# MasterVVK/qwen3-tts-axera-russian

Measured on AMD Instinct MI355X. Metric: 12Hz codec-tokens/s (codec frames/s, 16 codes each) + RTF, Qwen3-TTS-0.6B, higher is better.
Workload: dtype f16 weights/KV, f32 accumulate (talker+CP); vocoder exact fp32 (f32 MFMA); 1 GPU; configs[2]/[3]: batch=32 mixed ru/en prompts per GPU, 64 frames/utterance/step (prefill + hipGraph decode loop), utterance-sharded DP over 1 GPU(s); batch_per_gpu=32

## Files before the change

include/qwen3tts_engine.h:

```cpp
#ifndef QWEN3TTS_ENGINE_H
#define QWEN3TTS_ENGINE_H

#include <stdint.h>

#ifdef __cplusplus
extern "C" {
#endif

int q3_device_count(void);
int q3_device_compute_units(void);
int q3_set_device(int device);

void* q3e_create(const char* weights, int max_batch, int n_ctx, int max_frames);
void q3e_free(void* e);

int q3e_set_sampling(void* e, float talker_temperature, int talker_top_k, float talker_top_p,
                     float cp_temperature, int cp_top_k, uint64_t seed);

int q3e_set_forced_codes(void* e, const int32_t* forced, int n_frames);

int q3e_set_chains(void* e, int n);

int q3e_set_pad_embed(void* e, const float* pad_embed );

int q3e_start(void* e, int B, const float* prefix, const int32_t* n_rows, const int32_t* n_text,
              int ignore_eos, int max_frames);

int q3e_run(void* e, int n_frames);

float q3e_last_run_ms(void* e);
float q3e_last_prefill_ms(void* e);

int q3e_get_codes(void* e, int32_t* out, int max_out_frames, int32_t* n_frames_per_utt);

int q3e_get_done(void* e, int32_t* done , int32_t* frames );
int q3e_refill(void* e, int n, const int32_t* slots, const float* prefix, const int32_t* n_rows, const int32_t* n_text);

typedef struct q3e_slot_params {
    int32_t max_frames;
    float temperature;
    int32_t top_k;
    float top_p;
    float cp_temperature;
    int32_t cp_top_k;
    uint64_t seed;
    int32_t utt;
    int32_t reserved;
} q3e_slot_params;

int q3e_open(void* e, int B, int ignore_eos);
int q3e_admit(void* e, int n, const int32_t* slots, const float* prefix, const int32_t* n_rows, const int32_t* n_text,
              const q3e_slot_params* params);
int q3e_release(void* e, int n, const int32_t* slots);

int q3e_get_hidden(void* e, float* out);

double q3e_step_weight_bytes(void* e);

#ifdef __cplusplus
}
#endif
#endif
```

qwen3_tts_axera_russian_amd/build.py:

```python
from __future__ import annotations

import os
import shutil
import subprocess
import sys

HERE = os.path.dirname(os.path.abspath(__file__))
CSRC = os.path.join(HERE, "csrc")
LIB = os.path.join(HERE, "lib")
SOURCES = ["q3_common.cpp", "q3_formats.cpp", "q3_kernels.hip", "q3_model.hip", "q3_talker_api.hip", "q3_cp_api.hip",
           "q3_engine.hip", "q3_voc_kernels.hip", "q3_voc.hip", "q3_voc_stream.hip", "q3_enc.hip", "q3_enc_stream.hip",
           "q3_text_api.hip"]
TEST_SOURCES = ["q3_test_api.hip"]
ARCH = os.environ.get("Q3_OFFLOAD_ARCH", "gfx950")
EXTRA = os.environ.get("Q3_EXTRA_HIPCC_FLAGS", "-mllvm -amdgpu-kernarg-preload-count=16").split()


def _newer(dst: str, srcs) -> bool:
    if not os.path.exists(dst):
        return False
    t = os.path.getmtime(dst)
    return all(os.path.getmtime(s) <= t for s in srcs)


NO_SPILL = ("resunit_kernel", "linear_kernelILi1ELi1E", "linear_kernelILi1ELi2E", "linear_kernelILi2ELi1E",
            "linear_kernelILi2ELi2E", "attn_kernel", "attn_short_kernel", "cp_argmax_kernel", "talker_sample_kernel",
            "voc_attn_incr_kernel", "voc_incr_prepend_kernel", "voc_incr_emit_kernel", "voc_incr_prepend_split_kernel",
            "enc_stream_conv_in_kernel", "enc_stream_unfold_kernel", "enc_stream_emit_kernel")


def kernel_resources(lib_path: str):
    import re
    import struct
    import tempfile
    readelf = "/opt/rocm/lib/llvm/bin/llvm-readelf"
    d = open(lib_path, "rb").read()
    res = {}
    i = d.find(b"__CLANG_OFFLOAD_BUNDLE__")
    while i >= 0:
        n = struct.unpack_from("<Q", d, i + 24)[0]
        off = i + 32
        for _ in range(n):
            o, sz, ts = struct.unpack_from("<QQQ", d, off)
            off += 24
            triple = d[off:off + ts].decode()
            off += ts
            if ARCH in triple and sz:
                with tempfile.NamedTemporaryFile(suffix=".elf") as f:
                    f.write(d[i + o:i + o + sz])
                    f.flush()
                    notes = subprocess.run([readelf, "--notes", f.name], capture_output=True, text=True).stdout
                for blk in re.split(r"\n\s+- \.agpr_count:", notes)[1:]:
                    def g(key, blk=blk):
                        m = re.search(r"\." + key + r":\s+(\S+)", blk)
                        return m.group(1) if m else "0"
                    res[g("name")] = (int(g("vgpr_count")), int(blk.split()[0]), int(g("vgpr_spill_count")),
                                      int(g("private_segment_fixed_size")))
        i = d.find(b"__CLANG_OFFLOAD_BUNDLE__", i + 1)
    return res


def check_spills(lib_path: str, verbose: bool = False) -> None:
    if not os.path.exists("/opt/rocm/lib/llvm/bin/llvm-readelf"):
        return
    bad, others = [], []
    for name, (v, a, spill, scratch) in sorted(kernel_resources(lib_path).items()):
        if spill:
            (bad if any(k in name for k in NO_SPILL) else others).append(f"{name}: {spill} spilled VGPRs ({scratch} B scratch)")
    if verbose and others:
        print("kernels with spilled registers (not on the no-spill list):\n  " + "\n  ".join(others), flush=True)
    if bad:
        raise RuntimeError("register spills in kernels that must not spill:\n  " + "\n  ".join(bad))


def build(force: bool = False, verbose: bool = False, timeline: bool = False, refresh_timeline: bool = True) -> str:
    os.makedirs(LIB, exist_ok=True)
    hipcc = shutil.which("hipcc") or "/opt/rocm/bin/hipcc"
    srcs = [os.path.join(CSRC, s) for s in SOURCES if os.path.exists(os.path.join(CSRC, s))]
    hdrs = [os.path.join(CSRC, f) for f in os.listdir(CSRC) if f.endswith(".h")]
    hdrs += [os.path.join(HERE, "..", "include", f) for f in os.listdir(os.path.join(HERE, "..", "include"))]
    tag = "_tl" if timeline else ""
    out = os.path.join(LIB, f"libqwen3tts{tag}.so")
    objs, jobs = [], []
    for s in srcs:
        o = os.path.join(LIB, os.path.basename(s) + tag + ".o")
        objs.append(o)
        if not force and _newer(o, [s] + hdrs):
            continue
        jobs.append([hipcc, f"--offload-arch={ARCH}", "-O3", "-std=c++17", "-fPIC", "-x", "hip", "-c", s, "-o", o,
                     "-Wno-unused-result", "-Wno-unused-value", "-Wno-pass-failed"] + (["-DQ3_TIMELINE"] if timeline else []) + EXTRA)

    def run(cmd):
        if verbose:
            print(" ".join(cmd), flush=True)
        subprocess.check_call(cmd)

    if jobs:
        from concurrent.futures import ThreadPoolExecutor
        with ThreadPoolExecutor(max_workers=min(4, len(jobs))) as pool:
            list(pool.map(run, jobs))
    if force or not _newer(out, objs):
        cmd = [hipcc, f"--offload-arch={ARCH}", "-shared", "-fPIC", "-o", out] + objs + ["-lz"]
        if verbose:
            print(" ".join(cmd), flush=True)
        subprocess.check_call(cmd)
    tout = os.path.join(LIB, f"libqwen3tts_test{tag}.so")
    tsrcs = [os.path.join(CSRC, s) for s in TEST_SOURCES]
    if force or not _newer(tout, tsrcs + hdrs + [out]):
        cmd = [hipcc, f"--offload-arch={ARCH}", "-O3", "-std=c++17", "-fPIC", "-shared", "-x", "hip"] + tsrcs + \
# ... 26 lines not shown
```

qwen3_tts_axera_russian_amd/csrc/q3_cp.h:

```cpp
#pragma once
#include "q3_model.h"

namespace q3 {

struct CpFrameIO {
    int* codes = nullptr;
    const int* n_frames = nullptr;
    int frame_cap = 1;
    float* fb_h = nullptr;
    float* fb_ssq = nullptr;
    half_t* fb_xh = nullptr;
    const float* fb_gamma = nullptr;
    const float* pad_embed = nullptr;
    float temperature = 0.f;
    int top_k = 50;
    unsigned long long seed = 0;
    const unsigned long long* seed_ptr = nullptr;
    const int* forced = nullptr;
    const SlotParams* slots = nullptr;
};

int cp_seed_row0(const Work& w, int R, int row0 = 0, int R_total = 0);
int cp_frame(hipStream_t s, const Model& m, Work& w, KVCache& kv, int R, const CpFrameIO& io, int row0 = 0,
             int R_total = 0);

}
```

qwen3_tts_axera_russian_amd/csrc/q3_cp_api.hip:

```cpp
#include "../../include/qwen3tts_cp.h"
#include "q3_cp.h"

namespace q3 {

static bool two_row_enabled() {
    static const bool on = !(getenv("Q3_CP_TWO_ROW") && atoi(getenv("Q3_CP_TWO_ROW")) == 0);
    return on;
}

int cp_seed_row0(const Work& w, int R, int row0, int R_total) {
    (void)R;
    (void)row0;
    if (R_total <= 0) R_total = R;
    const int B16 = (R_total + 15) / 16 * 16;
    const bool two = two_row_enabled() && 2 * B16 <= w.max_rows;
    return two ? B16 : 0;
}

int cp_frame(hipStream_t s, const Model& m, Work& w, KVCache& kv, int R, const CpFrameIO& io, int row0, int R_total) {
    const ModelCfg& c = m.cfg;
    if (R_total <= 0) R_total = R;
    const int H = c.hidden, G = c.cp_groups;
    const int seed0 = cp_seed_row0(w, R, row0, R_total);
    RowMap rm;
    rm.slot_base = 0;
    rm.slot_stride = 1;
    rm.pos_stride = 0;
    if (seed0 > 0 && (row0 != 0 || R_total != R)) {
        RowMap r0;
        r0.slot_base = -seed0;
        r0.slot_stride = 1;
        r0.pos_base = 0;
        r0.pos_stride = 0;
        r0.same_slot_rows = true;
        if (run_stack(s, m, m.cp, w, kv, R, r0, 256, seed0 + row0)) return -1;
        if (launch_gather_embed(s, m.talker_emb, c.talker_vocab, H, io.codes, 0, io.n_frames, io.frame_cap, 0, w.h, w.ssq, R,
                                row0, R_total, io.forced, w.xh, m.cp.L[0].in_ln))
            return -1;
        RowMap r1 = rm;
        r1.pos_base = 1;
        r1.same_slot_rows = true;
        if (run_stack(s, m, m.cp, w, kv, R, r1, 256, row0)) return -1;
    } else if (seed0 > 0) {
        const int R16 = seed0;
        if (w.map_R16 != R16) {
            std::vector<int> slot(2 * R16), pos(2 * R16);
            for (int i = 0; i < 2 * R16; i++) {
                slot[i] = i % R16;
                pos[i] = i < R16 ? 1 : 0;
            }
            Q3_HIP(hipMemcpyAsync(w.map_slot, slot.data(), sizeof(int) * 2 * R16, hipMemcpyHostToDevice, s), -1);
            Q3_HIP(hipMemcpyAsync(w.map_pos, pos.data(), sizeof(int) * 2 * R16, hipMemcpyHostToDevice, s), -1);
            Q3_HIP(hipStreamSynchronize(s), -1);
            w.map_R16 = R16;
        }
        if (launch_gather_embed(s, m.talker_emb, c.talker_vocab, H, io.codes, 0, io.n_frames, io.frame_cap, 0, w.h, w.ssq, R,
                                row0, R_total, io.forced, w.xh, m.cp.L[0].in_ln))
            return -1;
        RowMap r2;
        r2.slot = w.map_slot;
        r2.pos = w.map_pos;
        r2.same_slot_rows = true;
        r2.valid_mod = R16;
        r2.valid_n = R;
        if (run_stack(s, m, m.cp, w, kv, R16 + R, r2, 256, 0)) return -1;
    } else {
        rm.pos_base = 0;
        if (run_stack(s, m, m.cp, w, kv, R, rm, 256, row0)) return -1;
        if (launch_gather_embed(s, m.talker_emb, c.talker_vocab, H, io.codes, 0, io.n_frames, io.frame_cap, 0, w.h, w.ssq, R,
                                row0, R_total, io.forced, w.xh, m.cp.L[0].in_ln))
            return -1;
        rm.pos_base = 1;
        if (run_stack(s, m, m.cp, w, kv, R, rm, 256, row0)) return -1;
    }
    const bool qkv_tab = m.cp_qkv_serves(R);
    for (int g = 0; g < G; g++) {
        if (g > 0) {
            rm.pos_base = g + 1;
            rm.skip_qkv0 = qkv_tab;
            if (run_stack(s, m, m.cp, w, kv, R, rm, 256, row0)) return -1;
        }
        LinArgs a;
        a.wp = m.cp_head[g].wp;
        a.N = c.cp_vocab;
        a.K = H;
        a.M = row0 + R;
        a.m_begin = row0;
        a.nt = 0;
        a.x16 = w.xh;
        a.ssq = w.ssq;
        a.ssq_parts = H / 16;
        a.eps = c.eps;
        a.y = w.logits;
        a.ldy = c.cp_vocab;
        if (launch_linear(s, a, PRO_NORM, EPI_STORE)) return -1;
        CpArgmaxArgs x;
        x.logits = w.logits;
        x.V = c.cp_vocab;
        x.R = R;
        x.row0 = row0;
        x.R_total = R_total;
        x.H = H;
        x.group = g;
        x.codes = io.codes;
        x.n_frames = io.n_frames;
        x.frame_cap = io.frame_cap;
        x.temperature = io.temperature;
        x.top_k = io.top_k;
        x.seed = io.seed;
        x.seed_ptr = io.seed_ptr;
        x.forced = io.forced;
        x.slots = io.slots;
        if (g + 1 < G) {
            x.next_table = m.cp_emb[g];
            x.h_out = w.h;
            x.ssq_out = w.ssq;
            x.xh_out = w.xh;
            x.gamma_next = m.cp.L[0].in_ln;
            if (qkv_tab) {
                x.next_qkv = m.cp_qkv_rows(g);
                x.qkv_out = w.qkv;
                x.qkv_ld = (c.n_heads + 2 * c.n_kv) * c.head_dim;
            }
        } else if (io.fb_h) {
            x.talker_emb = m.talker_emb;
            x.talker_vocab = c.talker_vocab;
            x.cp_tables = m.d_cp_emb_ptrs;
            x.pad_embed = io.pad_embed;
            x.n_groups = G;
            x.h_out = io.fb_h;
            x.ssq_out = io.fb_ssq;
            x.xh_out = io.fb_xh;
            x.gamma_next = io.fb_gamma;
        }
        if (launch_cp_argmax(s, x)) return -1;
    }
    return 0;
}

}

using namespace q3;

namespace {

struct CpHandle {
    Model* m = nullptr;
    int max_batch = 1;
    KVCache kv;
    Work w;
    hipStream_t s = nullptr;
    int *d_codes = nullptr, *d_nframes = nullptr;
    std::vector<int> h_codes;
    GraphExec graph;
    int graph_rows = 0;
    int step_next_pos = 0;
};

}

extern "C" {

void* cp_load(const char* weights, const char* embeddings_dir, int max_batch) {
    if (!weights) return nullptr;
    if (max_batch <= 0) max_batch = 1;
    hipStream_t s = nullptr;
    if (hipStreamCreate(&s) != hipSuccess) return nullptr;
    Model* m = model_load(weights, false, true, embeddings_dir, s);
    if (!m) {
        hipStreamDestroy(s);
        return nullptr;
    }
    CpHandle* h = new CpHandle();
    h->m = m;
    h->s = s;
    h->max_batch = max_batch;
    const ModelCfg& c = m->cfg;
    bool ok = kv_alloc(h->kv, c.cp_layers, max_batch, c.n_kv, c.cp_groups + 1, h->s) == 0;
// ... 143 lines not shown
```

qwen3_tts_axera_russian_amd/csrc/q3_engine.hip:

```cpp
#include "../../include/qwen3tts_engine.h"
#include "q3_cp.h"

#include <algorithm>
#include <chrono>
#include <cmath>

using namespace q3;

namespace {

struct Engine {
    Model* m = nullptr;
    int max_batch = 0, n_ctx = 0, max_frames = 0;
    hipStream_t s = nullptr;
    KVCache kv_t, kv_c;
    Work wt, wc;
    int prefill_rows = 0;
    int *d_slot = nullptr, *d_pos = nullptr;
    int* d_tiles = nullptr;
    int *d_iota = nullptr;
    int *d_past = nullptr, *d_npast = nullptr, *d_ntext = nullptr, *d_done = nullptr, *d_nframes = nullptr;
    int *d_pos0 = nullptr, *d_posdec = nullptr, *d_lastrow = nullptr;
    int* d_codes = nullptr;
    int* d_forced = nullptr;
// ... 28 lines not shown
    unsigned long long z = seed + golden * k;
    z = (z ^ (z >> 30)) * 0xBF58476D1CE4E5B9ull;
    z = (z ^ (z >> 27)) * 0x94D049BB133111EBull;
    return z ^ (z >> 31);
}

int talker_tail(Engine* e, hipStream_t st, int row0, int R) {
    const Model& m = *e->m;
    const int H = m.cfg.hidden;
    FinalNormArgs f;
    f.h = e->wt.h;
    f.ssq = e->wt.ssq;
    f.ssq_parts = H / 16;
    f.gamma = m.talker.final_norm;
    f.eps = m.cfg.eps;
    f.R = R;
    f.row0 = row0;
    f.H = H;
    f.out_f32 = e->wt.hidden_f32;
    f.out_f16 = e->wt.hidden_f16;
    f.out_copy = e->wc.h;
    f.out_copy_ssq = e->wc.ssq;
    f.out_copy_xh = e->wc.xh;
    f.out_copy_gamma = m.cp.L[0].in_ln;
    f.out_copy_row_off = cp_seed_row0(e->wc, R, row0, e->B);
    if (launch_final_norm(st, f)) return -1;
    LinArgs a;
    a.wp = m.talker_head.wp;
    a.N = m.cfg.talker_vocab;
    a.K = H;
    a.M = row0 + R;
    a.m_begin = row0;
    a.nt = 1;
    a.x16 = e->wt.hidden_f16;
    a.y = e->wt.logits;
    a.ldy = m.cfg.talker_vocab;
    return launch_linear(st, a, PRO_F16, EPI_STORE);
}

int frame_chain(Engine* e, hipStream_t st, int row0, int R) {
    const Model& m = *e->m;
    TalkerSampleArgs sa;
    sa.logits = e->wt.logits;
    sa.V = m.cfg.talker_vocab;
    sa.R = R;
    sa.row0 = row0;
    sa.R_total = e->B;
    sa.audio_vocab = m.cfg.cp_vocab;
    sa.eos = m.cfg.codec_eos;
    sa.past = e->d_past;
    sa.n_past = e->d_npast;
    sa.n_text = e->d_ntext;
    sa.done = e->d_done;
    sa.codes = e->d_codes;
    sa.n_frames = e->d_nframes;
    sa.frame_cap = e->max_frames;
    sa.pos0 = e->d_pos0;
    sa.pos = e->d_posdec;
    sa.ignore_eos = e->ignore_eos;
    sa.max_frames = e->cap_frames;
    sa.temperature = e->t_temp;
    sa.top_k = e->t_top_k;
    sa.top_p = e->t_top_p;
    sa.seed = e->seed;
    sa.seed_ptr = e->d_seed;
    sa.forced = e->forced_on ? e->d_forced : nullptr;
    sa.slots = e->slot_mode ? e->d_slots : nullptr;
    if (launch_talker_sample(st, sa)) return -1;
    CpFrameIO io;
    io.codes = e->d_codes;
    io.n_frames = e->d_nframes;
    io.frame_cap = e->max_frames;
    io.fb_h = e->wt.h;
    io.fb_ssq = e->wt.ssq;
    io.fb_xh = e->wt.xh;
    io.fb_gamma = m.talker.L[0].in_ln;
    io.pad_embed = e->d_pad;
    io.temperature = e->c_temp;
    io.top_k = e->c_top_k;
    io.seed = e->seed ^ 0x5851F42D4C957F2Dull;
    io.seed_ptr = e->d_seed;
    io.forced = e->forced_on ? e->d_forced : nullptr;
    io.slots = e->slot_mode ? e->d_slots : nullptr;
    if (cp_frame(st, m, e->wc, e->kv_c, R, io, row0, e->B)) return -1;
    RowMap rm;
    rm.slot_base = 0;
    rm.slot_stride = 1;
    rm.pos = e->d_posdec;
    rm.rows_total = e->B;
    if (run_stack(st, m, m.talker, e->wt, e->kv_t, R, rm, 1024, row0)) return -1;
    return talker_tail(e, st, row0, R);
}

int n_chains_eff(const Engine* e) {
    const int nc = e->n_chains < 1 ? 1 : e->n_chains;
    return (nc > 1 && e->B % (16 * nc) == 0) ? nc : 1;
}

void chain_rows(const Engine* e, int c, int& row0, int& R) {
    const int nc = n_chains_eff(e);
    row0 = 0;
    for (int i = 0; i < c; i++) row0 += e->B / nc + (i < e->B % nc ? 1 : 0);
    R = e->B / nc + (c < e->B % nc ? 1 : 0);
}

bool make_stream(const Engine* e, hipStream_t* st) {
    return (e->use_prio ? hipStreamCreateWithPriority(st, hipStreamNonBlocking, e->prio_hi)
                        : hipStreamCreateWithFlags(st, hipStreamNonBlocking)) == hipSuccess;
}

int ensure_chains(Engine* e, int n) {
    if (n < 2) return 0;
    if (!e->ev_fork) Q3_HIP(hipEventCreateWithFlags(&e->ev_fork, hipEventDisableTiming), -1);
    for (int c = 0; c < n; c++) {
        if (!e->cs[c] && !make_stream(e, &e->cs[c])) return -1;
        if (!e->ev_join[c]) Q3_HIP(hipEventCreateWithFlags(&e->ev_join[c], hipEventDisableTiming), -1);
    }
    return 0;
}

hipStream_t chain_stream(const Engine* e, int c) { return n_chains_eff(e) == 1 ? e->s : e->cs[c]; }

int frame_eager(Engine* e) {
    const int nc = n_chains_eff(e);
    for (int c = 0; c < nc; c++) {
        int row0, R;
        chain_rows(e, c, row0, R);
        if (frame_chain(e, chain_stream(e, c), row0, R)) return -1;
    }
    return 0;
}

int fork_chains(Engine* e) {
    const int nc = n_chains_eff(e);
    if (nc == 1) return 0;
    Q3_HIP(hipEventRecord(e->ev_fork, e->s), -1);
    for (int c = 0; c < nc; c++) Q3_HIP(hipStreamWaitEvent(e->cs[c], e->ev_fork, 0), -1);
    return 0;
}
int join_chains(Engine* e) {
    const int nc = n_chains_eff(e);
    if (nc == 1) return 0;
    for (int c = 0; c < nc; c++) {
        Q3_HIP(hipEventRecord(e->ev_join[c], e->cs[c]), -1);
        Q3_HIP(hipStreamWaitEvent(e->s, e->ev_join[c], 0), -1);
    }
    return 0;
}

}

extern "C" {

void q3e_free(void* ee) {
    Engine* e = (Engine*)ee;
    if (!e) return;
    if (e->s) hipStreamSynchronize(e->s);
    for (auto& g : e->graph) g.reset();
    kv_free(e->kv_t);
    kv_free(e->kv_c);
    work_free(e->wt);
    work_free(e->wc);
    void* ps[] = {e->d_tiles, e->d_slot, e->d_pos,  e->d_iota,   e->d_past,    e->d_npast, e->d_ntext, e->d_done,
                  e->d_nframes, e->d_pos0, e->d_posdec, e->d_lastrow, e->d_codes, e->d_pad, e->d_forced, e->d_seed, e->d_slots};
    for (void* p : ps)
        if (p) hipFree(p);
// ... 287 lines not shown
    Q3_HIP(hipStreamSynchronize(e->s), -1);
    hipEventElapsedTime(&e->last_prefill_ms, e->ev0, e->ev1);
    return 0;
}

int q3e_run(void* ee, int n_frames) {
    Engine* e = (Engine*)ee;
    if (!e || e->B <= 0 || n_frames <= 0) return -1;
    int room = (e->cap_frames < e->max_frames ? e->cap_frames : e->max_frames) - e->frames_run;
    if (e->slot_mode) {
        room = 0;
        for (int b = 0; b < e->B; b++)
            if (e->h_live[b]) room = std::max(room, e->h_budget[b] - e->h_age[b]);
    }
    if (room <= 0) return 0;
    if (n_frames > room) n_frames = room;
    int done_frames = 0;
    const int nc = n_chains_eff(e);
    Q3_HIP(hipEventRecord(e->ev0, e->s), -1);
    if (fork_chains(e)) return -1;
    static const bool no_graph = getenv("Q3_NO_GRAPH") && atoi(getenv("Q3_NO_GRAPH")) != 0;
    const bool need_capture = !e->graph[0].e || e->graph_B != e->B || e->graph_ignore != e->ignore_eos ||
                              e->graph_cap != e->cap_frames || e->graph_chains != nc ||
                              e->graph_slots != (int)e->slot_mode;
    if (no_graph) {
        for (; done_frames < n_frames; done_frames++)
            if (frame_eager(e)) return -1;
    } else if (need_capture) {
        if (frame_eager(e)) return -1;
        done_frames++;
        for (int c = 0; c < nc; c++) Q3_HIP(hipStreamSynchronize(chain_stream(e, c)), -1);
        for (int c = 0; c < nc; c++) {
            int row0, R;
            chain_rows(e, c, row0, R);
            e->graph[c].reset();
            Q3_HIP(hipStreamBeginCapture(chain_stream(e, c), hipStreamCaptureModeRelaxed), -1);
            int rc = frame_chain(e, chain_stream(e, c), row0, R);
            hipError_t er = hipStreamEndCapture(chain_stream(e, c), &e->graph[c].g);
            if (rc || er != hipSuccess) {
                Q3_LOG("q3e_run: graph capture failed");
                return -1;
            }
            Q3_HIP(hipGraphInstantiate(&e->graph[c].e, e->graph[c].g, nullptr, nullptr, 0), -1);
        }
        e->graph_B = e->B;
        e->graph_ignore = e->ignore_eos;
        e->graph_cap = e->cap_frames;
        e->graph_chains = nc;
        e->graph_slots = (int)e->slot_mode;
    }
    const int check_every = 16;
    const auto th0 = std::chrono::steady_clock::now();
    while (!no_graph && done_frames < n_frames) {
        int chunk = n_frames - done_frames;
        if (!e->ignore_eos && chunk > check_every) chunk = check_every;
        for (int i = 0; i < chunk; i++)
            for (int c = 0; c < nc; c++) Q3_HIP(hipGraphLaunch(e->graph[c].e, chain_stream(e, c)), -1);
        done_frames += chunk;
        if (!e->ignore_eos && done_frames < n_frames) {
            if (join_chains(e)) return -1;
            Q3_HIP(hipMemcpyAsync(e->h_done, e->d_done, sizeof(int) * e->B, hipMemcpyDeviceToHost, e->s), -1);
            Q3_HIP(hipStreamSynchronize(e->s), -1);
            bool all = true;
            for (int b = 0; b < e->B; b++) all = all && e->h_done[b];
            if (all) break;
            if (fork_chains(e)) return -1;
        }
    }
    e->last_host_launch_ms = (float)std::chrono::duration<double, std::milli>(std::chrono::steady_clock::now() - th0).count();
    if (join_chains(e)) return -1;
    Q3_HIP(hipEventRecord(e->ev1, e->s), -1);
    Q3_HIP(hipStreamSynchronize(e->s), -1);
    hipEventElapsedTime(&e->last_run_ms, e->ev0, e->ev1);
    if (e->slot_mode) {
        for (int b = 0; b < e->B; b++)
            if (e->h_age[b] >= 0) e->h_age[b] = std::min(e->h_age[b] + done_frames, e->max_frames);
        return done_frames;
    }
    e->frames_run += done_frames;
    e->frames_hi += done_frames;
    return done_frames;
}

float q3e_last_run_ms(void* ee) { return ee ? ((Engine*)ee)->last_run_ms : -1.f; }
float q3e_last_host_launch_ms(void* ee) { return ee ? ((Engine*)ee)->last_host_launch_ms : -1.f; }
float q3e_last_prefill_ms(void* ee) { return ee ? ((Engine*)ee)->last_prefill_ms : -1.f; }

int q3e_get_codes(void* ee, int32_t* out, int max_out_frames, int32_t* n_frames_per_utt) {
    Engine* e = (Engine*)ee;
    if (!e || !out || e->B <= 0) return -1;
    int nf = e->frames_hi < e->max_frames ? e->frames_hi : e->max_frames;
    if (e->slot_mode) {
        int hi = 0;
        for (int b = 0; b < e->B; b++)
            hi = std::max(hi, e->h_age[b]);
        nf = std::min(hi, e->max_frames);
    }
    if (nf > max_out_frames) nf = max_out_frames;
    int* h_np = e->h_read;
    int* h_codes = e->h_read + e->max_batch;
    const size_t n_codes = 16 * (size_t)e->B * (nf > 0 ? nf : 0);
    if (n_codes) Q3_HIP(hipMemcpyAsync(h_codes, e->d_codes, sizeof(int) * n_codes, hipMemcpyDeviceToHost, e->s), -1);
    if (n_frames_per_utt) Q3_HIP(hipMemcpyAsync(h_np, e->d_npast, sizeof(int) * e->B, hipMemcpyDeviceToHost, e->s), -1);
    Q3_HIP(hipStreamSynchronize(e->s), -1);
    if (n_codes) memcpy(out, h_codes, sizeof(int) * n_codes);
    if (n_frames_per_utt) memcpy(n_frames_per_utt, h_np, sizeof(int) * e->B);
    return nf;
}

int q3e_get_done(void* ee, int32_t* done, int32_t* frames) {
    Engine* e = (Engine*)ee;
    if (!e || !done || e->B <= 0) return -1;
    Q3_HIP(hipMemcpyAsync(e->h_done, e->d_done, sizeof(int) * e->B, hipMemcpyDeviceToHost, e->s), -1);
    Q3_HIP(hipMemcpyAsync(e->h_read, e->d_npast, sizeof(int) * e->B, hipMemcpyDeviceToHost, e->s), -1);
    Q3_HIP(hipStreamSynchronize(e->s), -1);
    memcpy(done, e->h_done, sizeof(int) * e->B);
    std::vector<int> np(e->h_read, e->h_read + e->B);
    for (int b = 0; b < e->B; b++)
        if (np[b] >= (e->slot_mode ? e->h_budget[b] : e->cap_frames)) done[b] = 1;
    if (e->slot_mode)
        for (int b = 0; b < e->B; b++)
            if (done[b]) e->h_live[b] = 0;
    if (frames) memcpy(frames, np.data(), sizeof(int) * e->B);
    return 0;
}

int q3e_refill(void* ee, int n, const int32_t* slots, const float* prefix, const int32_t* n_rows, const int32_t* n_text) {
    Engine* e = (Engine*)ee;
    if (!e || e->B <= 0 || n <= 0 || n > e->B || !slots || !prefix || !n_rows || !n_text) return -1;
    if (e->forced_on) {
        Q3_LOG("q3e_refill: a teacher-forced batch cannot be refilled");
        return -1;
    }
    if (e->slot_mode) {
        Q3_LOG("q3e_refill: a per-slot batch (q3e_open) takes new utterances with q3e_admit");
        return -1;
    }
    std::vector<int> ids(slots, slots + n), seen(e->B, 0);
    for (int u = 0; u < n; u++) {
        const int b = ids[u];
        if (b < 0 || b >= e->B || seen[b]++) {
            Q3_LOG("q3e_refill: slot %d is out of range or listed twice (batch of %d)", b, e->B);
            return -1;
        }
        if (n_rows[u] <= 0 || n_rows[u] > e->prefill_rows || n_rows[u] + e->cap_frames > e->n_ctx) {
            Q3_LOG("q3e_refill: utterance %d: %d prefix rows + %d frames do not fit n_ctx=%d", u, n_rows[u], e->cap_frames, e->n_ctx);
            return -1;
        }
    }
    Q3_HIP(hipStreamSynchronize(e->s), -1);
    Q3_HIP(hipEventRecord(e->ev0, e->s), -1);
    for (int u = 0; u < n; u++) {
        const int b = ids[u];
        if (clear_slot(e, b, n_rows + u, n_text + u)) return -1;
        unsigned long long z = e->req_seed + 0xD1B54A32D192ED03ull * ++e->n_refills;
        z = (z ^ (z >> 30)) * 0xBF58476D1CE4E5B9ull;
        z = (z ^ (z >> 27)) * 0x94D049BB133111EBull;
        z ^= z >> 31;
        Q3_HIP(hipMemcpyAsync(e->d_seed + b, &z, sizeof(z), hipMemcpyHostToDevice, e->s), -1);
        Q3_HIP(hipStreamSynchronize(e->s), -1);
    }
    Q3_HIP(hipStreamSynchronize(e->s), -1);
    if (prefill_ids(e, n, ids.data(), prefix, n_rows, e->B)) return -1;
    if (head_all_rows(e)) return -1;
    Q3_HIP(hipEventRecord(e->ev1, e->s), -1);
    Q3_HIP(hipStreamSynchronize(e->s), -1);
// ... 150 lines not shown
```

qwen3_tts_axera_russian_amd/csrc/q3_kernels.h:

```cpp
#pragma once
#include "q3_common.h"

namespace q3 {

enum { PRO_F16 = 0, PRO_NORM = 1 };
enum { EPI_STORE = 0, EPI_RESID = 1, EPI_SWIGLU = 2 };

struct LinArgs {
    int tl_node = -1;
    const half_t* wp = nullptr;
    int N = 0, K = 0, M = 0;
    int m_begin = 0;
    int swap_grid = 0;
    int nt = 0;
    const half_t* x16 = nullptr;
    const float* ssq = nullptr;
    int ssq_parts = 0;
    float eps = 1e-6f;
    float* y = nullptr;
    int ldy = 0;
    float* h_out = nullptr;
    float* ssq_out = nullptr;
    half_t* xh_out = nullptr;
    const float* gamma = nullptr;
    half_t* act = nullptr;
};
int launch_linear(hipStream_t s, const LinArgs& a, int pro, int epi);
int linear_decode_kbw(int K, int N, int rows);

int launch_pack_linear(hipStream_t s, const half_t* src, int N, int K, half_t* dst, int tile_off,
                       int tile_stride);

enum { ATTN_FUSED = 0, ATTN_PREP = 1, ATTN_ATTEND = 2 };
struct AttnArgs {
    int tl_node = -1;
    float* qkv = nullptr;
    int ld = 0, R = 0, row0 = 0;
    const float* q_norm = nullptr;
    const float* k_norm = nullptr;
    float eps = 1e-6f;
    const float* rope_cos = nullptr;
    const float* rope_sin = nullptr;
    const int* slot = nullptr;
    const int* pos = nullptr;
    int slot_base = 0, slot_stride = 0, pos_base = 0, pos_stride = 0;
    half_t* kc = nullptr;
    half_t* vc = nullptr;
    int n_ctx = 0, n_kv = 0, n_heads = 0;
    half_t* out = nullptr;
    float scale = 0.f;
    int threads = 256;
    int valid_mod = 0, valid_n = 0;
    const int* tiles = nullptr;
    int n_tiles = 0;
};
int launch_attn(hipStream_t s, const AttnArgs& a, int mode);

int launch_ssq_rows(hipStream_t s, const float* rows, float* h, float* ssq, int R, int H, half_t* xh = nullptr,
                    const float* gamma = nullptr, int dst_row0 = 0);

struct FinalNormArgs {
    int tl_node = -1;
    const float* h = nullptr;
    const float* ssq = nullptr;
    int ssq_parts = 0;
    const float* gamma = nullptr;
    float eps = 1e-6f;
    int R = 0, H = 0, row0 = 0;
    const int* row_map = nullptr;
    int src_off = 0;
    float* out_f32 = nullptr;
    half_t* out_f16 = nullptr;
    float* out_copy = nullptr;
    float* out_copy_ssq = nullptr;
    int out_copy_row_off = 0;
    half_t* out_copy_xh = nullptr;
    const float* out_copy_gamma = nullptr;
};
int launch_final_norm(hipStream_t s, const FinalNormArgs& a);

int launch_gather_embed(hipStream_t s, const float* table, int V, int H, const int* tok, int tok_stride,
                        const int* n_frames, int frame_cap, int col, float* h, float* ssq, int R, int row0 = 0,
                        int R_total = 0, const int* forced = nullptr, half_t* xh = nullptr, const float* gamma = nullptr);

struct SlotParams {
    int max_frames = 0;
    float t_temp = 0.f;
    int t_top_k = 0;
    float t_top_p = 1.f;
    float c_temp = 0.f;
    int c_top_k = 0;
    unsigned long long seed = 0;
    int no_row = 1;
    int pad_ = 0;
};

struct TalkerSampleArgs {
    int tl_node = -1;
    const float* logits = nullptr;
    int V = 0, R = 0, row0 = 0, R_total = 0;
    int audio_vocab = 2048, eos = 2150;
    int* past = nullptr;
    int* n_past = nullptr;
    const int* n_text = nullptr;
    int* done = nullptr;
    int* codes = nullptr;
    int* n_frames = nullptr;
    int frame_cap = 0;
    const int* pos0 = nullptr;
    int* pos = nullptr;
    int ignore_eos = 0;
    int max_frames = 0;
    float rep_penalty = 1.2f;
    float temperature = 0.f, top_p = 0.95f;
    int top_k = 50;
    unsigned long long seed = 0;
    const unsigned long long* seed_ptr = nullptr;
    const int* forced = nullptr;
    const SlotParams* slots = nullptr;
};
int launch_talker_sample(hipStream_t s, const TalkerSampleArgs& a);

struct CpArgmaxArgs {
    int tl_node = -1;
    const float* logits = nullptr;
    int V = 0, R = 0, H = 0, row0 = 0, R_total = 0;
    int group = 0;
    int* codes = nullptr;
    const int* n_frames = nullptr;
    int frame_cap = 0;
    const float* next_table = nullptr;
    float* h_out = nullptr;
    float* ssq_out = nullptr;
    half_t* xh_out = nullptr;
    const float* gamma_next = nullptr;
    const float* next_qkv = nullptr;
    float* qkv_out = nullptr;
    int qkv_ld = 0;
// ... 22 lines not shown
```

qwen3_tts_axera_russian_amd/csrc/q3_kernels.hip:

```cpp
#include "q3_kernels.h"

namespace q3 {

typedef _Float16 h8 __attribute__((ext_vector_type(8)));
typedef float f4 __attribute__((ext_vector_type(4)));

#ifdef Q3_TIMELINE
__device__ unsigned long long* g_tl = nullptr;
__device__ unsigned int g_tl_idx = 0;
__device__ unsigned int g_tl_cap = 0;
__device__ int g_skip = 0;
__device__ unsigned long long* g_ph = nullptr;
struct TlScope {
    unsigned int slot = 0xffffffffu;
    int id;
    __device__ __forceinline__ TlScope(int id_) : id(id_) {
        if (blockIdx.x == 0 && blockIdx.y == 0 && threadIdx.x == 0 && g_tl) {
            slot = atomicAdd(&g_tl_idx, 1u);
            if (slot < g_tl_cap) g_tl[2 * slot] = (wall_clock64() << 8) | (unsigned)id;
        }
    }
    __device__ __forceinline__ ~TlScope() {
        if (slot < g_tl_cap) g_tl[2 * slot + 1] = wall_clock64();
    }
};
__device__ unsigned long long* g_tl2 = nullptr;
__device__ int* g_tl2_kind = nullptr;
constexpr int TL2_MAXB = 1024;
struct TlScope2 {
    unsigned long long t0;
    int node, kind;
    __device__ __forceinline__ TlScope2(int n, int k) : node(n), kind(k) { t0 = wall_clock64(); }
    __device__ __forceinline__ ~TlScope2() {
        if (g_tl2 && node >= 0 && threadIdx.x == 0) {
            const unsigned b = blockIdx.x + gridDim.x * blockIdx.y;
            if (b < TL2_MAXB) {
                g_tl2[((size_t)node * TL2_MAXB + b) * 2] = t0;
                g_tl2[((size_t)node * TL2_MAXB + b) * 2 + 1] = wall_clock64();
            }
            if (b == 0 && g_tl2_kind) g_tl2_kind[node] = kind;
        }
    }
};
#define Q3_TL(id)      \
    if (g_skip) return; \
    TlScope2 tl_scope2_(a.tl_node, id); \
    TlScope tl_scope_(id)
#define Q3_PH(n)                                                                                       \
    do {                                                                                               \
        if (tl_scope_.slot < g_tl_cap && g_ph) g_ph[(size_t)tl_scope_.slot * 8 + (n)] = wall_clock64(); \
    } while (0)
#else
#ifndef Q3_WAVE_PRIO
#define Q3_WAVE_PRIO 3
#endif
#if Q3_WAVE_PRIO > 0
#define Q3_TL(id) __builtin_amdgcn_s_setprio(Q3_WAVE_PRIO)
#else
#define Q3_TL(id)
#endif
#define Q3_PH(n)
#endif

#define Q3_FETCH_ARGS(...) asm volatile("" ::__VA_ARGS__)

__device__ __forceinline__ int uniform_load(const int* p) {
    return *(const __attribute__((address_space(4))) int*)p;
}

__device__ __forceinline__ float wave_sum(float v) {
#pragma unroll
    for (int o = 32; o > 0; o >>= 1) v += __shfl_xor(v, o, 64);
    return v;
}
__device__ __forceinline__ float wave_max(float v) {
#pragma unroll
    for (int o = 32; o > 0; o >>= 1) v = fmaxf(v, __shfl_xor(v, o, 64));
    return v;
}
__device__ __forceinline__ half_t sat_half(float x) {
    return (half_t)fminf(fmaxf(x, -65504.f), 65504.f);
}
constexpr float NORM_PRE = 0.0625f, NORM_POST = 16.0f;
#ifdef Q3_NT_OUT
#define Q3_OUT_STORE(v_, p_) __builtin_nontemporal_store((v_), (p_))
#else
#define Q3_OUT_STORE(v_, p_) (*(p_) = (v_))
#endif
__device__ __forceinline__ half_t pre_scaled(float h, float g) { return sat_half((h * g) * NORM_PRE); }

__device__ __forceinline__ size_t frag_idx(int m, int k, int K) {
    return ((((size_t)(m >> 4) * (K >> 5) + (k >> 5)) * 64 + (m & 15) + 16 * ((k >> 3) & 3)) << 3) + (k & 7);
}

__global__ void pack_linear_kernel(const half_t* __restrict__ src, int N, int K, half_t* __restrict__ dst,
                                   int tile_off, int tile_stride) {
    const int KB = K / 32;
    size_t idx = (size_t)blockIdx.x * blockDim.x + threadIdx.x;
    size_t total = (size_t)(N / 16) * KB * 64;
    if (idx >= total) return;
    int lane = (int)(idx & 63);
    size_t blk = idx >> 6;
    int kb = (int)(blk % KB);
    int ts = (int)(blk / KB);
    int n = ts * 16 + (lane & 15);
    int k = kb * 32 + (lane >> 4) * 8;
    h8 v = *(const h8*)(src + (size_t)n * K + k);
    size_t td = (size_t)tile_off + (size_t)ts * tile_stride;
    *(h8*)(dst + ((td * KB + kb) * 64 + lane) * 8) = v;
}

int launch_pack_linear(hipStream_t s, const half_t* src, int N, int K, half_t* dst, int tile_off,
                       int tile_stride) {
    if (N % 16 || K % 32) {
        Q3_LOG("pack_linear: N=%d K=%d not multiples of 16/32", N, K);
        return -1;
    }
    size_t total = (size_t)(N / 16) * (K / 32) * 64;
    int blocks = (int)((total + 255) / 256);
    hipLaunchKernelGGL(pack_linear_kernel, dim3(blocks), dim3(256), 0, s, src, N, K, dst, tile_off, tile_stride);
    Q3_HIP(hipGetLastError(), -1);
    return 0;
}

static const char* g_last_variant = "";
const char* last_linear_variant() { return g_last_variant; }
static const char* pro_name(int pro) { return pro == PRO_NORM ? "NORM" : "F16"; }
static const char* epi_name(int epi) { return epi == EPI_STORE ? "STORE" : epi == EPI_RESID ? "RESID" : "SWIGLU"; }
static int env_int(const char* name, int dflt) { return getenv(name) ? atoi(getenv(name)) : dflt; }

template <int NB16, int MT16, int KBW, int NW, int PRO, int EPI, bool NT>
__global__ void __launch_bounds__(NW * 64)
    linear_kernel(const half_t* __restrict__ p_wp, const void* __restrict__ p_asrc, const float* __restrict__ p_ssq,
                  const float* __restrict__ p_gamma, void* __restrict__ p_out, int p_M, int p_N, int p_m_begin,
                  int p_swap, float p_eps, LinArgs a) {
    a.wp = p_wp;
    a.x16 = (const half_t*)p_asrc;
    a.ssq = p_ssq;
    a.gamma = p_gamma;
    a.y = (float*)p_out;
    a.h_out = (float*)p_out;
    a.act = (half_t*)p_out;
    a.M = p_M;
    a.N = p_N;
    a.m_begin = p_m_begin;
    a.swap_grid = p_swap;
    a.eps = p_eps;
    constexpr int MR = MT16 * 16, NB = NB16 * 16, NBP = NB + 4, KB = NW * KBW, K = KB * 32;
    constexpr int NTH = NW * 64;
    constexpr int NOUT = (EPI == EPI_SWIGLU) ? MR * NB / 2 : MR * NB;
    constexpr int OPT = (NOUT + NTH - 1) / NTH;
    constexpr int SQI = (MR * 16 + NTH - 1) / NTH;
    Q3_TL(10 + PRO * 4 + EPI);
    const int tid = threadIdx.x, lane = tid & 63, w = tid >> 6;
    const int q = lane >> 4, c = lane & 15;
    const int tile0 = (a.swap_grid ? blockIdx.y : blockIdx.x) * NB16;
    const int m0 = a.m_begin + (a.swap_grid ? blockIdx.x : blockIdx.y) * MR;
    extern __shared__ __attribute__((aligned(16))) char smem[];
    float* red = (float*)smem;
    float* inv_s = red + NW * MR * NBP;

    float4 sq[SQI];
    h8 af[MT16][KBW];
    float hold[OPT], gnext[OPT];
    if (PRO == PRO_NORM) {
#pragma unroll
        for (int i = 0; i < SQI; i++) {
            const int g4 = tid + i * NTH, g4c = g4 < MR * 16 ? g4 : 0;
            sq[i] = *(const float4*)(a.ssq + (size_t)(m0 + g4c / 16) * 64 + (g4c & 15) * 4);
        }
    }
    if (EPI == EPI_RESID) {
#pragma unroll
        for (int i = 0; i < OPT; i++) {
            const int o = tid + i * NTH;
            const int m = m0 + o / NB;
            hold[i] = 0.f;
            gnext[i] = 0.f;
            if (o < NOUT && m < a.M) hold[i] = a.h_out[frag_idx(m, tile0 * 16 + (o % NB), a.N)];
            if (o < NOUT && a.gamma) gnext[i] = a.gamma[tile0 * 16 + (o % NB)];
        }
    }
    h8 wf[NB16][KBW];
#pragma unroll
    for (int nb = 0; nb < NB16; nb++)
#pragma unroll
        for (int kbi = 0; kbi < KBW; kbi++) {
            const h8* p = (const h8*)(a.wp + (((size_t)(tile0 + nb) * KB + (size_t)w * KBW + kbi) * 64 + lane) * 8);
            wf[nb][kbi] = NT ? __builtin_nontemporal_load(p) : *p;
        }
#pragma unroll
    for (int kbi = 0; kbi < KBW; kbi++) {
        const int k0 = (w * KBW + kbi) * 32 + q * 8;
#pragma unroll
        for (int mt = 0; mt < MT16; mt++) {
            af[mt][kbi] = *(const h8*)(a.x16 + frag_idx(m0 + mt * 16 + c, k0, K));
        }
    }
    __builtin_amdgcn_sched_barrier(0);
    if (EPI == EPI_RESID) Q3_FETCH_ARGS("s"(a.ssq_out), "s"(a.xh_out));
    if (EPI == EPI_STORE) Q3_FETCH_ARGS("s"(a.ldy));
    if (PRO == PRO_NORM) Q3_FETCH_ARGS("s"(a.eps));
    Q3_PH(0);

    if (PRO == PRO_NORM) {
#pragma unroll
        for (int i = 0; i < SQI; i++) {
            const int g4 = tid + i * NTH;
            float s = (sq[i].x + sq[i].y) + (sq[i].z + sq[i].w);
            s += __shfl_xor(s, 8, 16);
            s += __shfl_xor(s, 4, 16);
            s += __shfl_xor(s, 2, 16);
            s += __shfl_xor(s, 1, 16);
            if (g4 < MR * 16 && (g4 & 15) == 0) inv_s[g4 / 16] = (1.0f / sqrtf(s / (float)K + a.eps)) * NORM_POST;
        }
    }

    Q3_PH(1);
    f4 acc[MT16][NB16];
#pragma unroll
    for (int mt = 0; mt < MT16; mt++)
#pragma unroll
        for (int nb = 0; nb < NB16; nb++) acc[mt][nb] = (f4){0.f, 0.f, 0.f, 0.f};
#pragma unroll
    for (int kbi = 0; kbi < KBW; kbi++)
#pragma unroll
        for (int mt = 0; mt < MT16; mt++)
#pragma unroll
            for (int nb = 0; nb < NB16; nb++)
                acc[mt][nb] = __builtin_amdgcn_mfma_f32_16x16x32_f16(af[mt][kbi], wf[nb][kbi], acc[mt][nb], 0, 0, 0);

    asm volatile("" ::"v"(acc[0][0][0]));
    Q3_PH(2);
#define RED(w_, row_, col_) red[((w_) * MR + (row_)) * NBP + (col_)]
#pragma unroll
    for (int mt = 0; mt < MT16; mt++)
#pragma unroll
        for (int nb = 0; nb < NB16; nb++)
#pragma unroll
            for (int r = 0; r < 4; r++) RED(w, mt * 16 + 4 * q + r, nb * 16 + c) = acc[mt][nb][r];
    __syncthreads();
    Q3_PH(3);

    if (EPI == EPI_STORE || EPI == EPI_RESID) {
#pragma unroll
        for (int i = 0; i < OPT; i++) {
            const int o = tid + i * NTH;
            if (o < NOUT) {
                const int mr = o / NB, n = o % NB;
                float v = 0.f;
#pragma unroll
                for (int ww = 0; ww < NW; ww++) v += RED(ww, mr, n);
                const int m = m0 + mr;
                const int ng = tile0 * 16 + n;
                const bool ok = m < a.M;
                if (PRO == PRO_NORM) v *= inv_s[mr];
                if (EPI == EPI_STORE) {
                    if (ok) Q3_OUT_STORE(v, &a.y[(size_t)m * a.ldy + ng]);
                } else {
                    const float hn = ok ? hold[i] + v : 0.f;
                    if (ok) Q3_OUT_STORE(hn, &a.h_out[frag_idx(m, ng, a.N)]);
                    if (ok && a.xh_out) Q3_OUT_STORE(pre_scaled(hn, gnext[i]), &a.xh_out[frag_idx(m, ng, a.N)]);
                    float s = hn * hn;
                    s += __shfl_xor(s, 8, 16);
                    s += __shfl_xor(s, 4, 16);
                    s += __shfl_xor(s, 2, 16);
                    s += __shfl_xor(s, 1, 16);
                    if (ok && (n & 15) == 0) Q3_OUT_STORE(s, &a.ssq_out[(size_t)m * (a.N / 16) + (ng >> 4)]);
                }
            }
        }
    } else {
        constexpr int NH = NB / 2;
#pragma unroll
        for (int i = 0; i < OPT; i++) {
            const int o = tid + i * NTH;
            if (o < NOUT) {
                const int mr = o / NH, j = o % NH;
                const int ii = j >> 4, cc = j & 15;
                float g = 0.f, u = 0.f;
#pragma unroll
                for (int ww = 0; ww < NW; ww++) {
                    g += RED(ww, mr, (2 * ii) * 16 + cc);
                    u += RED(ww, mr, (2 * ii + 1) * 16 + cc);
                }
                const int m = m0 + mr;
                if (PRO == PRO_NORM) {
                    g *= inv_s[mr];
                    u *= inv_s[mr];
                }
                if (m < a.M) {
                    const float sg = __fdividef(g, 1.0f + __expf(-g));
                    Q3_OUT_STORE(sat_half(sg * u), &a.act[frag_idx(m, (tile0 / NB16) * NH + j, a.N / 2)]);
                }
            }
        }
    }
#undef RED
}

template <int NB16, int MT16, int KBW, int NW, int PRO, int EPI, bool NT>
static int launch_linear_nt(hipStream_t s, const LinArgs& a) {
    constexpr int MR = MT16 * 16, NBP = NB16 * 16 + 4;
    constexpr size_t lds = (size_t)NW * MR * NBP * 4 + MR * 4;
    static bool attr_set = false;
    if (!attr_set) {
        if (lds > 48 * 1024)
            Q3_HIP(hipFuncSetAttribute((const void*)linear_kernel<NB16, MT16, KBW, NW, PRO, EPI, NT>,
                                       hipFuncAttributeMaxDynamicSharedMemorySize, (int)lds), -1);
        attr_set = true;
    }
    static char name[64];
    if (!name[0])
        snprintf(name, sizeof(name), "linear<%d,%d,%d,%d,%s,%s,%s>", NB16, MT16, KBW, NW, pro_name(PRO), epi_name(EPI), NT ? "nt" : "t");
    g_last_variant = name;
    LinArgs b = a;
    b.tl_node = tl_next_node();
    const unsigned nt_ = a.N / (16 * NB16), nr_ = (a.M - a.m_begin + MR - 1) / MR;
    b.swap_grid = nr_ > 2 ? 1 : 0;
    dim3 grid(b.swap_grid ? nr_ : nt_, b.swap_grid ? nt_ : nr_);
    const void* asrc = (const void*)b.x16;
    void* outp = EPI == EPI_STORE ? (void*)b.y : EPI == EPI_RESID ? (void*)b.h_out : (void*)b.act;
    hipLaunchKernelGGL((linear_kernel<NB16, MT16, KBW, NW, PRO, EPI, NT>), grid, dim3(NW * 64), lds, s, b.wp, asrc, b.ssq,
                       b.gamma, outp, b.M, b.N, b.m_begin, b.swap_grid, b.eps, b);
    Q3_HIP(hipGetLastError(), -1);
    return 0;
}

__device__ __forceinline__ void gemm_tile_of_block(int R, int T, int& row_tile, int& col_tile) {
    const int L = blockIdx.x;
    if (T % 8 == 0) {
        const int x = L & 7, j = L >> 3;
        row_tile = j % R;
        col_tile = x + 8 * (j / R);
    } else {
        row_tile = L % R;
        col_tile = L / R;
    }
}

template <int BM, int BN, int PRO, int EPI>
__device__ __forceinline__ void gemm_epilogue(const LinArgs& a, f4 (&acc)[BM / 32][BN / 32], const float* post, int m0,
                                              int tile0, int wm, int wn, int q, int c) {
    constexpr int WM = BM / 32, WN = BN / 32;
#pragma unroll
    for (int i = 0; i < WM; i++) {
#pragma unroll
        for (int r = 0; r < 4; r++) {
            const int mr = (wm * WM + i) * 16 + 4 * q + r;
            const int m = m0 + mr;
            const bool ok = m < a.M;
            const float ps = PRO == PRO_NORM ? post[mr] : 1.0f;
            if (EPI == EPI_SWIGLU) {
#pragma unroll
                for (int j = 0; j < WN; j += 2) {
                    const float g = acc[i][j][r] * ps, u = acc[i][j + 1][r] * ps;
                    const float sg = __fdividef(g, 1.0f + __expf(-g));
                    const int jn = ((tile0 + wn * WN + j) >> 1) * 16 + c;
                    if (ok) a.act[frag_idx(m, jn, a.N / 2)] = sat_half(sg * u);
                }
            } else {
#pragma unroll
                for (int j = 0; j < WN; j++) {
                    const int ng = (tile0 + wn * WN + j) * 16 + c;
                    const float v = acc[i][j][r] * ps;
                    if (EPI == EPI_STORE) {
                        if (ok) a.y[(size_t)m * a.ldy + ng] = v;
                    } else {
                        const size_t hi = frag_idx(m, ng, a.N);
                        const float hn = ok ? a.h_out[hi] + v : 0.f;
                        if (ok) a.h_out[hi] = hn;
                        if (ok && a.xh_out) a.xh_out[hi] = pre_scaled(hn, a.gamma[ng]);
                        float s2 = hn * hn;
                        s2 += __shfl_xor(s2, 8, 16);
                        s2 += __shfl_xor(s2, 4, 16);
                        s2 += __shfl_xor(s2, 2, 16);
                        s2 += __shfl_xor(s2, 1, 16);
                        if (ok && c == 0) a.ssq_out[(size_t)m * (a.N / 16) + (ng >> 4)] = s2;
                    }
                }
            }
        }
    }
}

template <int BM, int BN, int KS, int PRO, int EPI>
__global__ void __launch_bounds__(256) gemm_kernel(LinArgs a) {
    constexpr int RA = BM / 16, RB = BN / 16;
    constexpr int NF = (RA + RB) * KS, FPW = NF / 4;
    constexpr int WM = BM / 32, WN = BN / 32;
    static_assert(NF % 4 == 0 && WN % 2 == 0, "tile shape");
    Q3_TL(20 + PRO * 4 + EPI);
    const int tid = threadIdx.x, lane = tid & 63, w = tid >> 6;
    const int wm = w >> 1, wn = w & 1, q = lane >> 4, c = lane & 15;
    int row_tile, col_tile;
    gemm_tile_of_block((a.M - a.m_begin + BM - 1) / BM, a.N / BN, row_tile, col_tile);
    const int m0 = a.m_begin + row_tile * BM;
    const int tile0 = col_tile * RB;
    const int KB = a.K >> 5, NST = KB / KS;
    extern __shared__ __attribute__((aligned(16))) char smem[];
    h8* lds = (h8*)smem;
    __shared__ float post[BM];
    if (PRO == PRO_NORM) {
        for (int r = tid; r < BM; r += 256) {
            const int m = m0 + r;
// ... 302 lines not shown
        for (int kbi = 0; kbi < KBW; kbi++)
            af[kbi] = *(const h8*)(p_x16 + frag_idx(blk0 + c, (w * KBW + kbi) * 32 + q * 8, K));
    }
    __builtin_amdgcn_sched_barrier(0);
    Q3_PH(0);
    f4 acc = (f4){0.f, 0.f, 0.f, 0.f};
#pragma unroll
    for (int kbi = 0; kbi < KBW; kbi++) acc = __builtin_amdgcn_mfma_f32_16x16x32_f16(af[kbi], wf[kbi], acc, 0, 0, 0);
    Q3_PH(2);
    if ((q >> 1) == half) *(f4*)(red + ((w * 2 + (q & 1)) * 16 + c) * 4) = acc;
    __syncthreads();
    Q3_PH(3);
    if (epi_thread) {
        float v = 0.f;
#pragma unroll
        for (int ww = 0; ww < NW; ww++) v += red[((ww * 2 + (mr >> 2)) * 16 + n) * 4 + (mr & 3)];
        const float hn = ok ? hold + v : 0.f;
        if (ok) Q3_OUT_STORE(hn, &p_h[frag_idx(m, ng, N)]);
        if (ok && p_xh_out) Q3_OUT_STORE(pre_scaled(hn, gnext), &p_xh_out[frag_idx(m, ng, N)]);
        float s = hn * hn;
        s += __shfl_xor(s, 8, 16);
        s += __shfl_xor(s, 4, 16);
        s += __shfl_xor(s, 2, 16);
        s += __shfl_xor(s, 1, 16);
        if (ok && n == 0) Q3_OUT_STORE(s, &p_ssq_out[(size_t)m * (N / 16) + tile0]);
    }
}

static int g_narrow8 = env_int("Q3_LINEAR_NARROW8", 1);
int set_linear_narrow8(int on) { g_narrow8 = on; return 0; }

template <int KBW, int NW>
static int launch_linear_narrow_t(hipStream_t s, const LinArgs& a) {
    const int groups = (a.M - a.m_begin + 7) / 8;
    const int node = tl_next_node();
    static char name[2][32];
    if (!name[0][0]) {
        snprintf(name[0], sizeof(name[0]), "narrow<%d,%d,t>", KBW, NW);
        snprintf(name[1], sizeof(name[1]), "narrow<%d,%d,nt>", KBW, NW);
    }
    g_last_variant = name[a.nt ? 1 : 0];
    if (a.nt)
        hipLaunchKernelGGL((linear_narrow_kernel<KBW, NW, true>), dim3(64, groups), dim3(NW * 64), 0, s, a.wp, a.x16, a.h_out, a.gamma,
                           a.ssq_out, a.xh_out, a.M, a.m_begin, node);
    else
        hipLaunchKernelGGL((linear_narrow_kernel<KBW, NW, false>), dim3(64, groups), dim3(NW * 64), 0, s, a.wp, a.x16, a.h_out, a.gamma,
                           a.ssq_out, a.xh_out, a.M, a.m_begin, node);
    Q3_HIP(hipGetLastError(), -1);
    return 0;
}

#define Q3_LIN_CASE(NB16_, MT16_, KBW_, NW_, PRO_, EPI_)                                   \
    if (nb16 == NB16_ && mt16 == MT16_ && kbw == KBW_ && nw == NW_ && pro == PRO_ && epi == EPI_) \
        return launch_linear_t<NB16_, MT16_, KBW_, NW_, PRO_, EPI_>(s, a);

#define Q3_LIN_MT(NB16_, KBW_, NW_, PRO_, EPI_) \
    Q3_LIN_CASE(NB16_, 1, KBW_, NW_, PRO_, EPI_) \
    Q3_LIN_CASE(NB16_, 2, KBW_, NW_, PRO_, EPI_) \
    Q3_LIN_CASE(NB16_, 4, KBW_, NW_, PRO_, EPI_)

int reset_linear_knobs() {
    memcpy(g_tune_kbw, g_tune_kbw_default, sizeof(g_tune_kbw));
    g_wide_tiles = 0;
    g_split_rows_narrow = 1;
    g_gemm_min_rows = 65;
    g_narrow8 = env_int("Q3_LINEAR_NARROW8", 1);
    g_gemm_glds = env_int("Q3_GEMM_GLDS", 1);
    return 0;
}

static int decode_mt16(int rows, int N) {
    int mt16 = rows <= 16 ? 1 : rows <= 32 ? 2 : 4;
    if (rows > 16 && rows <= 32 && ((g_split_rows_narrow == 1 && N <= 1024) || g_split_rows_narrow == 2)) mt16 = 1;
    return mt16;
}

int linear_decode_kbw(int K, int N, int rows) {
    const int ki = K == 1024 ? 0 : K == 2048 ? 1 : K == 3072 ? 2 : -1;
    if (rows <= 0 || rows >= g_gemm_min_rows || ki < 0 || N % 32) return 0;
    const int mt16 = decode_mt16(rows, N);
    return g_tune_kbw[ki][mt16 == 1 ? 0 : mt16 == 2 ? 1 : 2];
}

int launch_linear(hipStream_t s, const LinArgs& a, int pro, int epi) {
    g_last_variant = "";
    const int rows = a.M - a.m_begin;
    if (rows <= 0) return 0;
    if (rows >= g_gemm_min_rows) return launch_gemm(s, a, pro, epi);
    const int K = a.K;
    int ki = K == 1024 ? 0 : K == 2048 ? 1 : K == 3072 ? 2 : -1;
    if (ki < 0 || a.N % 32) {
        Q3_LOG("launch_linear: unsupported shape N=%d K=%d", a.N, K);
        return -1;
    }
    if (g_narrow8 && pro == PRO_F16 && epi == EPI_RESID && a.N == 1024 && a.m_begin % 16 == 0 && a.ssq_out) {
        if (K == 2048) return launch_linear_narrow_t<16, 4>(s, a);
        if (K == 3072) return launch_linear_narrow_t<12, 8>(s, a);
    }
    const int mt16 = decode_mt16(rows, a.N);
    const int kbw = g_tune_kbw[ki][mt16 == 1 ? 0 : mt16 == 2 ? 1 : 2];
    const int nw = K / 32 / kbw;
    const int nb16 = (epi == EPI_SWIGLU || (g_wide_tiles && rows > 16 && K == 1024 && epi == EPI_STORE)) ? 2 : 1;
    Q3_LIN_MT(1, 8, 4, PRO_NORM, EPI_STORE)
    Q3_LIN_MT(1, 4, 8, PRO_NORM, EPI_STORE)
    Q3_LIN_MT(2, 8, 4, PRO_NORM, EPI_SWIGLU)
    Q3_LIN_MT(2, 4, 8, PRO_NORM, EPI_SWIGLU)
    Q3_LIN_MT(1, 8, 4, PRO_F16, EPI_STORE)
    Q3_LIN_MT(2, 4, 8, PRO_NORM, EPI_STORE)
    Q3_LIN_MT(2, 4, 8, PRO_F16, EPI_STORE)
    Q3_LIN_MT(1, 4, 8, PRO_F16, EPI_STORE)
    Q3_LIN_MT(1, 8, 8, PRO_F16, EPI_RESID)
    Q3_LIN_MT(1, 4, 16, PRO_F16, EPI_RESID)
    Q3_LIN_MT(1, 16, 4, PRO_F16, EPI_RESID)
    Q3_LIN_MT(1, 6, 16, PRO_F16, EPI_RESID)
    Q3_LIN_MT(1, 12, 8, PRO_F16, EPI_RESID)
    Q3_LOG("launch_linear: no instantiation for K=%d kbw=%d nw=%d mt16=%d nb16=%d pro=%d epi=%d", K, kbw, nw,
           mt16, nb16, pro, epi);
    return -1;
}

__device__ __forceinline__ void store_row_ssq(float* h, float* ssq, int r, int H, int k4, float4 v,
                                              half_t* xh = nullptr, const float* gamma = nullptr) {
    *(float4*)(h + frag_idx(r, k4 * 4, H)) = v;
    if (xh) {
        const float4 g = *(const float4*)(gamma + k4 * 4);
        half_t* p = xh + frag_idx(r, k4 * 4, H);
        p[0] = pre_scaled(v.x, g.x);
        p[1] = pre_scaled(v.y, g.y);
        p[2] = pre_scaled(v.z, g.z);
        p[3] = pre_scaled(v.w, g.w);
    }
    float s = v.x * v.x + v.y * v.y + v.z * v.z + v.w * v.w;
    s += __shfl_xor(s, 1, 4);
    s += __shfl_xor(s, 2, 4);
    if ((k4 & 3) == 0) ssq[(size_t)r * (H / 16) + (k4 >> 2)] = s;
}

__global__ void ssq_rows_kernel(const float* __restrict__ rows, float* __restrict__ h, float* __restrict__ ssq, int H,
                                half_t* __restrict__ xh, const float* __restrict__ gamma, int dst_row0) {
    const int r = blockIdx.x;
    for (int k4 = threadIdx.x; k4 < H / 4; k4 += blockDim.x)
        store_row_ssq(h, ssq, dst_row0 + r, H, k4, *(const float4*)(rows + (size_t)r * H + k4 * 4), xh, gamma);
}
int launch_ssq_rows(hipStream_t s, const float* rows, float* h, float* ssq, int R, int H, half_t* xh, const float* gamma,
                    int dst_row0) {
    if (R <= 0) return 0;
    hipLaunchKernelGGL(ssq_rows_kernel, dim3(R), dim3(256), 0, s, rows, h, ssq, H, xh, gamma, dst_row0);
    Q3_HIP(hipGetLastError(), -1);
    return 0;
}

__global__ void final_norm_kernel(FinalNormArgs a) {
    Q3_FETCH_ARGS("s"(a.h), "s"(a.ssq), "s"(a.ssq_parts), "s"(a.gamma), "s"(a.eps), "s"(a.H), "s"(a.row0), "s"(a.row_map), "s"(a.src_off),
                  "s"(a.out_f32), "s"(a.out_f16), "s"(a.out_copy), "s"(a.out_copy_ssq), "s"(a.out_copy_xh), "s"(a.out_copy_gamma),
                  "s"(a.out_copy_row_off));
    Q3_TL(40);
    __shared__ float inv_sh;
    const int r = a.row0 + blockIdx.x;
    const int src = a.row_map ? uniform_load(a.row_map + r) : r + a.src_off;
    if (threadIdx.x < 64) {
        float s = 0.f;
        for (int p = threadIdx.x; p < a.ssq_parts; p += 64) s += a.ssq[(size_t)src * a.ssq_parts + p];
        s = wave_sum(s);
        if (threadIdx.x == 0) inv_sh = 1.0f / sqrtf(s / (float)a.H + a.eps);
    }
    __syncthreads();
    const float iv = inv_sh;
    for (int k4 = threadIdx.x; k4 < a.H / 4; k4 += blockDim.x) {
        const float4 v = *(const float4*)(a.h + frag_idx(src, k4 * 4, a.H));
        const float4 g = *(const float4*)(a.gamma + k4 * 4);
        float4 o;
        o.x = (v.x * iv) * g.x;
        o.y = (v.y * iv) * g.y;
        o.z = (v.z * iv) * g.z;
        o.w = (v.w * iv) * g.w;
        if (a.out_f32) *(float4*)(a.out_f32 + (size_t)r * a.H + k4 * 4) = o;
        if (a.out_f16) {
            half_t* p = a.out_f16 + frag_idx(r, k4 * 4, a.H);
            p[0] = sat_half(o.x);
            p[1] = sat_half(o.y);
            p[2] = sat_half(o.z);
            p[3] = sat_half(o.w);
        }
        if (a.out_copy)
            store_row_ssq(a.out_copy, a.out_copy_ssq, r + a.out_copy_row_off, a.H, k4, o, a.out_copy_xh, a.out_copy_gamma);
    }
}
int launch_final_norm(hipStream_t s, const FinalNormArgs& a) {
    if (a.R <= 0) return 0;
    FinalNormArgs a2 = a;
    a2.tl_node = tl_next_node();
    hipLaunchKernelGGL(final_norm_kernel, dim3(a.R), dim3(256), 0, s, a2);
    Q3_HIP(hipGetLastError(), -1);
    return 0;
}

__global__ void gather_embed_kernel(const float* __restrict__ table, int V, int H, const int* __restrict__ tok,
                                    int tok_stride, const int* __restrict__ n_frames, int frame_cap, int col,
                                    float* __restrict__ h, float* __restrict__ ssq, int row0, int R_total,
                                    const int* __restrict__ forced, half_t* __restrict__ xh,
                                    const float* __restrict__ gamma) {
    const int r = row0 + blockIdx.x;
    int t;
// ... 152 lines not shown
        l1 = l1 * c1 + p1;
#pragma unroll
        for (int j = 0; j < 8; j++) {
            const float vf = (float)vv[j];
            a0[j] = a0[j] * c0 + p0 * vf;
            a1[j] = a1[j] * c1 + p1 * vf;
        }
        m0 = n0;
        m1 = n1;
    };
#pragma unroll
    for (int i = 0; i < APRE; i++) {
        const int t = grp + i * ngrp;
        if (t < T) step(kpre[i], vpre[i]);
    }
#pragma unroll 2
    for (int t = grp + APRE * ngrp; t < T; t += ngrp) {
        const h8 kk = *(const h8*)(kbase + (size_t)t * D + l16 * 8);
        const h8 vv = *(const h8*)(vbase + (size_t)t * D + l16 * 8);
        step(kk, vv);
    }
    if (MODE == ATTN_FUSED && grp == 0) {
        h8 kk, vv;
#pragma unroll
        for (int j = 0; j < 8; j++) {
            kk[j] = (half_t)knew[l16 * 8 + j];
            vv[j] = (half_t)vnew[l16 * 8 + j];
        }
        step(kk, vv);
    }
    asm volatile("" ::"v"(a0[0]), "v"(l0));
    Q3_PH(2);
#pragma unroll
    for (int o = 16; o <= 32; o <<= 1) {
        const float om0 = __shfl_xor(m0, o, 64), om1 = __shfl_xor(m1, o, 64);
        const float ol0 = __shfl_xor(l0, o, 64), ol1 = __shfl_xor(l1, o, 64);
        const float n0 = fmaxf(m0, om0), n1 = fmaxf(m1, om1);
        const float c0 = (m0 == -INFINITY) ? 0.f : __expf(m0 - n0), d0 = (om0 == -INFINITY) ? 0.f : __expf(om0 - n0);
        const float c1 = (m1 == -INFINITY) ? 0.f : __expf(m1 - n1), d1 = (om1 == -INFINITY) ? 0.f : __expf(om1 - n1);
        l0 = l0 * c0 + ol0 * d0;
        l1 = l1 * c1 + ol1 * d1;
#pragma unroll
        for (int j = 0; j < 8; j++) {
            const float oa0 = __shfl_xor(a0[j], o, 64), oa1 = __shfl_xor(a1[j], o, 64);
            a0[j] = a0[j] * c0 + oa0 * d0;
            a1[j] = a1[j] * c1 + oa1 * d1;
        }
        m0 = n0;
        m1 = n1;
    }
    if (lane < 16) {
#pragma unroll
        for (int j = 0; j < 8; j++) {
            pacc[(w * 2 + 0) * D + lane * 8 + j] = a0[j];
            pacc[(w * 2 + 1) * D + lane * 8 + j] = a1[j];
        }
        if (lane == 0) {
            pm[w * 2 + 0] = m0;
            pm[w * 2 + 1] = m1;
            pl[w * 2 + 0] = l0;
            pl[w * 2 + 1] = l1;
        }
    }
    __syncthreads();
    Q3_PH(3);
    if (tid < 2 * D) {
        const int hh = tid / D, d = tid % D;
        float M = -INFINITY;
        for (int i = 0; i < nwv; i++) M = fmaxf(M, pm[i * 2 + hh]);
        float L = 0.f, o = 0.f;
        for (int i = 0; i < nwv; i++) {
            const float mi = pm[i * 2 + hh];
            const float c = (mi == -INFINITY) ? 0.f : __expf(mi - M);
            L += pl[i * 2 + hh] * c;
            o += pacc[(i * 2 + hh) * D + d] * c;
        }
        a.out[frag_idx(r, (2 * g + hh) * D + d, a.n_heads * D)] = sat_half(o / L);
    }
}

constexpr int ATTN_SHORT_MAX_T = 15;
static int g_attn_short = 1;
int set_attn_short(int on) { g_attn_short = on; return 0; }
__global__ void __launch_bounds__(256)
    attn_short_kernel(float* __restrict__ p_qkv, int p_ld, int p_row0, int p_n_heads, int p_n_kv,
                      const float* __restrict__ p_q_norm, const float* __restrict__ p_k_norm,
                      const float* __restrict__ p_rope_cos, const float* __restrict__ p_rope_sin, int p_pos_base,
                      int p_slot_base, AttnArgs a) {
    constexpr int D = 128, NE = ATTN_SHORT_MAX_T + 1;
    a.qkv = p_qkv;
    a.ld = p_ld;
    a.row0 = p_row0;
    a.n_heads = p_n_heads;
    a.n_kv = p_n_kv;
    a.q_norm = p_q_norm;
    a.k_norm = p_k_norm;
    a.rope_cos = p_rope_cos;
    a.rope_sin = p_rope_sin;
    a.pos_base = p_pos_base;
    a.slot_base = p_slot_base;
    Q3_FETCH_ARGS("s"(a.eps), "s"(a.slot), "s"(a.slot_stride), "s"(a.kc), "s"(a.vc), "s"(a.n_ctx), "s"(a.out), "s"(a.scale));
    Q3_TL(33);
    const int r = a.row0 + blockIdx.x, g = blockIdx.y;
    const int tid = threadIdx.x, lane = tid & 63, w = tid >> 6;
    const int slot = a.slot ? uniform_load(a.slot + r) : a.slot_base + r * a.slot_stride;
    const int T = a.pos_base;
    __shared__ float qs[2][D];
    __shared__ float knew[D];
    __shared__ __attribute__((aligned(16))) half_t vs[NE][D];
    __shared__ __attribute__((aligned(16))) float sc[2][NE];
    float* row = a.qkv + (size_t)r * a.ld;
    const size_t cbase = ((size_t)slot * a.n_kv + g) * (size_t)a.n_ctx * D;
    const int l16 = tid & 15, grp = tid >> 4;
    const int hh = tid >> 7, d = tid & 127;
    float x0 = 0.f, x1 = 0.f, gm0 = 1.f, gm1 = 1.f, cs = 1.f, sn = 0.f;
    {
        const float* src = w < 2 ? row + (size_t)(2 * g + w) * D
                         : w == 2 ? row + (size_t)(a.n_heads + g) * D
                                  : row + (size_t)(a.n_heads + a.n_kv + g) * D;
        x0 = src[lane];
        x1 = src[lane + 64];
        if (w < 3) {
            const float* gam = w < 2 ? a.q_norm : a.k_norm;
            gm0 = gam[lane];
            gm1 = gam[lane + 64];
            cs = a.rope_cos[(size_t)T * 64 + lane];
            sn = a.rope_sin[(size_t)T * 64 + lane];
        }
    }
    h8 kpre, vpre;
    if (grp < T) {
        kpre = *(const h8*)(a.kc + cbase + (size_t)grp * D + l16 * 8);
        vpre = *(const h8*)(a.vc + cbase + (size_t)grp * D + l16 * 8);
    }
    __builtin_amdgcn_sched_barrier(0);
    Q3_PH(0);
    if (w < 3) {
        float ss = wave_sum(x0 * x0 + x1 * x1);
        const float iv = 1.0f / sqrtf(ss / (float)D + a.eps);
        x0 = (x0 * iv) * gm0;
        x1 = (x1 * iv) * gm1;
        const float y0 = x0 * cs - x1 * sn;
        const float y1 = x1 * cs + x0 * sn;
        x0 = y0;
        x1 = y1;
    }
    if (w < 2) {
        qs[w][lane] = x0;
        qs[w][lane + 64] = x1;
    } else {
        const half_t h0 = sat_half(x0), h1 = sat_half(x1);
        half_t* cd = (w == 2 ? a.kc : a.vc) + cbase + (size_t)T * D;
        cd[lane] = h0;
        cd[lane + 64] = h1;
        if (w == 2) {
            knew[lane] = (float)h0;
            knew[lane + 64] = (float)h1;
        } else {
            vs[T][lane] = h0;
            vs[T][lane + 64] = h1;
        }
    }
    if (grp < T) *(h8*)(&vs[grp][l16 * 8]) = vpre;
    __syncthreads();
    Q3_PH(1);
    if (grp <= T) {
        float d0 = 0.f, d1 = 0.f;
#pragma unroll
        for (int j = 0; j < 8; j++) {
            const float kf = grp < T ? (float)kpre[j] : knew[l16 * 8 + j];
            d0 += (qs[0][l16 * 8 + j] * a.scale) * kf;
            d1 += (qs[1][l16 * 8 + j] * a.scale) * kf;
        }
#pragma unroll
        for (int o = 8; o > 0; o >>= 1) {
            d0 += __shfl_xor(d0, o, 16);
            d1 += __shfl_xor(d1, o, 16);
        }
        if (l16 == 0) {
            sc[0][grp] = d0;
            sc[1][grp] = d1;
        }
    }
    __syncthreads();
    Q3_PH(2);
    float sv[NE];
#pragma unroll
    for (int e4 = 0; e4 < NE; e4 += 4) {
        const float4 t4 = *(const float4*)(&sc[hh][e4]);
        sv[e4] = t4.x;
        sv[e4 + 1] = t4.y;
        sv[e4 + 2] = t4.z;
        sv[e4 + 3] = t4.w;
    }
    float m = -INFINITY;
#pragma unroll
    for (int e = 0; e < NE; e++) m = fmaxf(m, e <= T ? sv[e] : -INFINITY);
    float L = 0.f, o = 0.f;
#pragma unroll
    for (int e = 0; e < NE; e++) {
        const float p = e <= T ? __expf(sv[e] - m) : 0.f;
        const float vf = e <= T ? (float)vs[e][d] : 0.f;
        L += p;
        o += p * vf;
    }
    Q3_PH(3);
    a.out[frag_idx(r, (2 * g + hh) * D + d, a.n_heads * D)] = sat_half(o / L);
}

__global__ void __launch_bounds__(256) attn_tile_mfma_kernel(AttnArgs a) {
    constexpr int D = 128, QP = 136, VP = 72, CH = 64;
    constexpr float LO = 2048.0f, ILO = 1.0f / 2048.0f;
    Q3_TL(35);
    const int g = blockIdx.y, tid = threadIdx.x, lane = tid & 63, w = tid >> 6;
    const int c = lane & 15, q4 = lane >> 4;
    int row0, nrows, slot, pos0;
    if (a.tiles) {
        const int4 t = *(const int4*)(a.tiles + 4 * blockIdx.x);
        row0 = t.x; nrows = t.y; slot = t.z; pos0 = t.w;
    } else {
        row0 = a.row0 + blockIdx.x * 16;
        nrows = a.R - blockIdx.x * 16 < 16 ? a.R - blockIdx.x * 16 : 16;
        slot = a.slot_base;
        pos0 = a.pos_base + blockIdx.x * 16;
    }
    extern __shared__ __attribute__((aligned(16))) char smem[];
    half_t* qh = (half_t*)smem;
    half_t* ql = qh + 32 * QP;
    half_t* ks = ql + 32 * QP;
    half_t* vs = ks + CH * QP;
    half_t* ph = vs + CH * QP;
    half_t* pl = ph + 32 * VP;
    float* red = (float*)(pl + 32 * VP);
    float* red2 = red + 4 * 32;
    const size_t cbase = ((size_t)slot * a.n_kv + g) * (size_t)a.n_ctx * D;
    const int T = pos0 + nrows;
    h8 kreg[4], vreg[4];
    auto load_chunk = [&](int c0) {
#pragma unroll
        for (int it = 0; it < 4; it++) {
            const int idx = tid + it * 256, kr = idx >> 4, d8 = (idx & 15) * 8;
            kreg[it] = vreg[it] = (h8){0, 0, 0, 0, 0, 0, 0, 0};
            if (c0 + kr < T) {
                kreg[it] = *(const h8*)(a.kc + cbase + (size_t)(c0 + kr) * D + d8);
                vreg[it] = *(const h8*)(a.vc + cbase + (size_t)(c0 + kr) * D + d8);
            }
        }
    };
    auto store_chunk = [&]() {
#pragma unroll
        for (int it = 0; it < 4; it++) {
            const int idx = tid + it * 256, kr = idx >> 4, d8 = (idx & 15) * 8;
            *(h8*)(ks + kr * QP + d8) = kreg[it];
            *(h8*)(vs + kr * QP + d8) = vreg[it];
        }
    };
    load_chunk(0);
    for (int idx = tid; idx < 32 * (D / 8); idx += 256) {
        const int qr = idx / (D / 8), d8 = (idx - qr * (D / 8)) * 8, i = qr & 15, hh = qr >> 4;
        h8 hi = {0, 0, 0, 0, 0, 0, 0, 0}, lo = hi;
        if (i < nrows) {
            const float* src = a.qkv + (size_t)(row0 + i) * a.ld + (size_t)(2 * g + hh) * D + d8;
            const float4 v0 = *(const float4*)src, v1 = *(const float4*)(src + 4);
            const float e[8] = {v0.x, v0.y, v0.z, v0.w, v1.x, v1.y, v1.z, v1.w};
#pragma unroll
            for (int j = 0; j < 8; j++) {
                const float x = e[j] * a.scale;
                hi[j] = sat_half(x);
                lo[j] = (half_t)((x - (float)hi[j]) * LO);
            }
        }
        *(h8*)(qh + qr * QP + d8) = hi;
        *(h8*)(ql + qr * QP + d8) = lo;
    }
    float mrow[2][4], lrow[2][4];
    f4 oh[2][2], ol[2][2];
#pragma unroll
    for (int qb = 0; qb < 2; qb++)
#pragma unroll
        for (int r = 0; r < 4; r++) {
            mrow[qb][r] = -INFINITY;
            lrow[qb][r] = 0.f;
        }
#pragma unroll
    for (int qb = 0; qb < 2; qb++)
#pragma unroll
        for (int j = 0; j < 2; j++) oh[qb][j] = ol[qb][j] = (f4){0.f, 0.f, 0.f, 0.f};
    for (int c0 = 0; c0 < T; c0 += CH) {
        __syncthreads();
        store_chunk();
// ... 31 lines not shown
                if (c == 0) red[w * 32 + 16 * qb + i] = x;
            }
        __syncthreads();
        float corr[2][4];
#pragma unroll
        for (int qb = 0; qb < 2; qb++)
#pragma unroll
            for (int r = 0; r < 4; r++) {
                const int qr = 16 * qb + 4 * q4 + r;
                const float cm = fmaxf(fmaxf(red[qr], red[32 + qr]), fmaxf(red[64 + qr], red[96 + qr]));
                const float mo = mrow[qb][r], mn = fmaxf(mo, cm);
                corr[qb][r] = (mo == -INFINITY) ? 0.f : __expf(mo - mn);
                const float p = (sc[qb][r] == -INFINITY) ? 0.f : __expf(sc[qb][r] - mn);
                const half_t hi = (half_t)p;
                ph[qr * VP + 16 * w + c] = hi;
                pl[qr * VP + 16 * w + c] = (half_t)((p - (float)hi) * LO);
                float ssum = p;
                ssum += __shfl_xor(ssum, 1, 16);
                ssum += __shfl_xor(ssum, 2, 16);
                ssum += __shfl_xor(ssum, 4, 16);
                ssum += __shfl_xor(ssum, 8, 16);
                if (c == 0) red2[w * 32 + qr] = ssum;
                mrow[qb][r] = mn;
            }
        __syncthreads();
#pragma unroll
        for (int qb = 0; qb < 2; qb++)
#pragma unroll
            for (int r = 0; r < 4; r++) {
                const int qr = 16 * qb + 4 * q4 + r;
                lrow[qb][r] = lrow[qb][r] * corr[qb][r] + ((red2[qr] + red2[32 + qr]) + (red2[64 + qr] + red2[96 + qr]));
#pragma unroll
                for (int j = 0; j < 2; j++) {
                    oh[qb][j][r] *= corr[qb][r];
                    ol[qb][j][r] *= corr[qb][r];
                }
            }
#pragma unroll
        for (int kst = 0; kst < 2; kst++) {
#pragma unroll
            for (int j = 0; j < 2; j++) {
                typedef __fp16 hv4 __attribute__((__vector_size__(4 * sizeof(__fp16))));
                const half_t* vb = vs + (kst * 32 + 8 * q4 + (c >> 2)) * QP + 32 * w + 16 * j + 4 * (c & 3);
                const hv4 t0 = __builtin_amdgcn_ds_read_tr16_b64_v4f16((__attribute__((address_space(3))) hv4*)vb);
                const hv4 t1 = __builtin_amdgcn_ds_read_tr16_b64_v4f16((__attribute__((address_space(3))) hv4*)(vb + 4 * QP));
                h8 bv;
#pragma unroll
                for (int e = 0; e < 4; e++) {
                    bv[e] = (half_t)t0[e];
                    bv[4 + e] = (half_t)t1[e];
                }
#pragma unroll
                for (int qb = 0; qb < 2; qb++) {
                    const h8 ahi = *(const h8*)(ph + (16 * qb + c) * VP + kst * 32 + q4 * 8);
                    const h8 alo = *(const h8*)(pl + (16 * qb + c) * VP + kst * 32 + q4 * 8);
                    oh[qb][j] = __builtin_amdgcn_mfma_f32_16x16x32_f16(ahi, bv, oh[qb][j], 0, 0, 0);
                    ol[qb][j] = __builtin_amdgcn_mfma_f32_16x16x32_f16(alo, bv, ol[qb][j], 0, 0, 0);
                }
            }
        }
    }
#pragma unroll
    for (int qb = 0; qb < 2; qb++)
#pragma unroll
        for (int r = 0; r < 4; r++) {
            const int i = 4 * q4 + r;
            if (i < nrows) {
                const float inv = 1.0f / lrow[qb][r];
#pragma unroll
                for (int j = 0; j < 2; j++) {
                    const float o = (oh[qb][j][r] + ol[qb][j][r] * ILO) * inv;
                    a.out[frag_idx(row0 + i, (2 * g + qb) * D + 32 * w + 16 * j + c, a.n_heads * D)] = sat_half(o);
                }
            }
        }
}

int launch_attn(hipStream_t s, const AttnArgs& a, int mode) {
    if (a.R <= 0) return 0;
    if (a.n_heads != 2 * a.n_kv) {
        Q3_LOG("attn: only GQA group 2 (16q/8kv) is built, got %d/%d", a.n_heads, a.n_kv);
        return -1;
    }
    if (g_attn_short && mode == ATTN_FUSED && !a.pos && a.pos_stride == 0 && a.pos_base >= 0 &&
        a.pos_base <= ATTN_SHORT_MAX_T && a.pos_base < a.n_ctx) {
        AttnArgs a3 = a;
        a3.tl_node = tl_next_node();
        hipLaunchKernelGGL(attn_short_kernel, dim3(a.R, a.n_kv), dim3(256), 0, s, a3.qkv, a3.ld, a3.row0, a3.n_heads, a3.n_kv,
                           a3.q_norm, a3.k_norm, a3.rope_cos, a3.rope_sin, a3.pos_base, a3.slot_base, a3);
        Q3_HIP(hipGetLastError(), -1);
        return 0;
    }
    if (mode == ATTN_ATTEND && a.n_tiles > 0) {
        constexpr size_t lds = (size_t)(2 * 32 * 136 + 2 * 64 * 136 + 2 * 32 * 72) * 2 + 8 * 32 * 4;
        static bool attr = false;
        if (!attr) {
            Q3_HIP(hipFuncSetAttribute((const void*)attn_tile_mfma_kernel, hipFuncAttributeMaxDynamicSharedMemorySize, (int)lds), -1);
            attr = true;
        }
        AttnArgs a5 = a;
        a5.tl_node = tl_next_node();
        hipLaunchKernelGGL(attn_tile_mfma_kernel, dim3(a.n_tiles, a.n_kv), dim3(256), lds, s, a5);
        Q3_HIP(hipGetLastError(), -1);
        return 0;
    }
    int threads = a.threads;
    const int fit = 65536 / (a.R * a.n_kv);
    if (threads > fit) threads = fit / 64 * 64;
    if (threads < 256) threads = 256;
    if (threads > 1024) threads = 1024;
    const size_t lds = ((size_t)(threads / 64) * (4 + 2 * 128)) * sizeof(float);
    AttnArgs a2 = a;
    a2.tl_node = tl_next_node();
    dim3 grid(a.R, a.n_kv);
#define Q3_ATTN(MODE_)                                                                                   \
    {                                                                                                    \
        if (threads <= 256)                                                                              \
            hipLaunchKernelGGL((attn_kernel<MODE_, 8>), grid, dim3(256), mode == ATTN_PREP ? 0 : lds, s, a2); \
        else                                                                                             \
            hipLaunchKernelGGL((attn_kernel<MODE_, 4>), grid, dim3(mode == ATTN_PREP ? 256 : threads),   \
                               mode == ATTN_PREP ? 0 : lds, s, a2);                                      \
    }
    if (mode == ATTN_FUSED) Q3_ATTN(ATTN_FUSED)
    else if (mode == ATTN_PREP) Q3_ATTN(ATTN_PREP)
    else Q3_ATTN(ATTN_ATTEND)
#undef Q3_ATTN
    Q3_HIP(hipGetLastError(), -1);
    return 0;
}

__device__ __forceinline__ void block_argmax(float& v, int& idx, float* sv, int* si) {
#pragma unroll
    for (int o = 32; o > 0; o >>= 1) {
        const float ov = __shfl_xor(v, o, 64);
        const int oi = __shfl_xor(idx, o, 64);
        if (ov > v || (ov == v && oi < idx)) {
            v = ov;
            idx = oi;
        }
    }
    const int w = threadIdx.x >> 6, nw = blockDim.x >> 6;
    if ((threadIdx.x & 63) == 0) {
        sv[w] = v;
        si[w] = idx;
    }
    __syncthreads();
    v = sv[0];
    idx = si[0];
    for (int i = 1; i < nw; i++)
        if (sv[i] > v || (sv[i] == v && si[i] < idx)) {
            v = sv[i];
            idx = si[i];
        }
    __syncthreads();
}

__device__ __forceinline__ float uniform01(unsigned long long seed, unsigned row, unsigned frame, unsigned group) {
    unsigned long long z = seed + 0x9E3779B97F4A7C15ull * (1ull + row + ((unsigned long long)frame << 20) +
                                                            ((unsigned long long)group << 44));
    z = (z ^ (z >> 30)) * 0xBF58476D1CE4E5B9ull;
    z = (z ^ (z >> 27)) * 0x94D049BB133111EBull;
    z = z ^ (z >> 31);
    return (float)(z >> 40) * (1.0f / 16777216.0f);
}

__device__ __forceinline__ float nan_as_inf(float l) { return l != l ? INFINITY : l; }

constexpr int SAMPLE_SEL_CAP = 64;
// ... 581 lines not shown
```

qwen3_tts_axera_russian_amd/csrc/q3_model.h:

```cpp
#pragma once
#include "q3_kernels.h"

namespace q3 {

struct DevLinear {
    half_t* wp = nullptr;
    int N = 0, K = 0;
};

struct DevLayer {
    DevLinear qkv, o, gu, down;
    float *in_ln = nullptr, *post_ln = nullptr, *q_norm = nullptr, *k_norm = nullptr;
};

struct DevStack {
    std::vector<DevLayer> L;
    float* final_norm = nullptr;
    const float* tail_gamma = nullptr;
    int ffn = 0;
    int nt = 0;
    size_t weight_bytes = 0;
};

struct Model {
    ModelCfg cfg;
    int device = 0;
    bool has_talker = false, has_cp = false;
    DevStack talker, cp;
    float* talker_emb = nullptr;
    DevLinear talker_head;
    std::vector<float*> cp_emb;
    std::vector<DevLinear> cp_head;
    const float** d_cp_emb_ptrs = nullptr;
    float* cp_qkv_tab = nullptr;
    int cp_qkv_kbw = 0;
    const float* cp_qkv_rows(int group) const {
        return cp_qkv_tab + (size_t)group * cfg.cp_vocab * ((cfg.n_heads + 2 * cfg.n_kv) * cfg.head_dim);
    }
    bool cp_qkv_serves(int rows) const {
        return cp_qkv_tab && linear_decode_kbw(cfg.hidden, (cfg.n_heads + 2 * cfg.n_kv) * cfg.head_dim, rows) == cp_qkv_kbw;
    }
    float *rope_cos = nullptr, *rope_sin = nullptr;
    int max_pos = 0;
    std::vector<void*> allocs;
    size_t device_bytes = 0;
};

Model* model_load(const char* path, bool want_talker, bool want_cp, const char* aux_dir = nullptr, hipStream_t s = nullptr);
void model_free(Model* m);

struct KVCache {
    half_t *k = nullptr, *v = nullptr;
    int n_layers = 0, n_slots = 0, n_kv = 0, n_ctx = 0, head_dim = 128;
    size_t layer_stride() const { return (size_t)n_slots * n_kv * n_ctx * head_dim; }
    size_t bytes() const { return layer_stride() * n_layers * sizeof(half_t) * 2; }
};
int kv_alloc(KVCache& kv, int n_layers, int n_slots, int n_kv, int n_ctx, hipStream_t s = nullptr);
void kv_free(KVCache& kv);
int kv_zero(hipStream_t s, KVCache& kv);

inline size_t frag_idx_host(int m, int k, int K) {
    return ((((size_t)(m >> 4) * (K >> 5) + (k >> 5)) * 64 + (m & 15) + 16 * ((k >> 3) & 3)) << 3) + (k & 7);
}

struct Work {
    int max_rows = 0, hidden = 0;
    float* rows_in = nullptr;
    float *h = nullptr, *ssq = nullptr, *qkv = nullptr;
    half_t* xh = nullptr;
    half_t *attn = nullptr, *act = nullptr;
    float* hidden_f32 = nullptr;
    half_t* hidden_f16 = nullptr;
    float* logits = nullptr;
    int *map_slot = nullptr, *map_pos = nullptr;
    int map_R16 = 0;
};
int work_alloc(Work& w, const ModelCfg& c, int max_rows, int ffn, int max_vocab, hipStream_t s = nullptr);
void work_free(Work& w);
int work_zero(hipStream_t s, Work& w, const ModelCfg& c, int ffn, int max_vocab);

struct RowMap {
    const int* slot = nullptr;
    const int* pos = nullptr;
    int slot_base = 0, slot_stride = 0, pos_base = 0, pos_stride = 0;
    bool same_slot_rows = false;
    int valid_mod = 0, valid_n = 0;
    const int* tiles = nullptr;
    int n_tiles = 0;
    bool skip_qkv0 = false;
    int rows_total = 0;
};

int run_stack(hipStream_t s, const Model& m, const DevStack& st, Work& w, KVCache& kv, int R,
              const RowMap& rm, int attn_threads, int row0 = 0);

struct GraphExec {
    hipGraph_t g = nullptr;
    hipGraphExec_t e = nullptr;
    void reset();
};

}
```

qwen3_tts_axera_russian_amd/csrc/q3_model.hip:

```cpp
#include "q3_model.h"

#include <cmath>

namespace q3 {

namespace {

struct Loader {
    Model* m;
    const Pack& p;
    hipStream_t s = nullptr;
    half_t* stage = nullptr;
    size_t stage_elems = 0;
    std::vector<uint16_t> host16;
    bool ok = true;

    bool up(void* d, const void* src, size_t bytes) {
        return hipMemcpyAsync(d, src, bytes, hipMemcpyHostToDevice, s) == hipSuccess && hipStreamSynchronize(s) == hipSuccess;
    }
    void* dalloc(size_t bytes) {
        void* d = nullptr;
        if (hipMalloc(&d, bytes) != hipSuccess) {
            Q3_LOG("hipMalloc(%zu) failed", bytes);
            ok = false;
// ... 249 lines not shown
            if (!L.up(m->rope_cos, cs.data(), cs.size() * 4)) L.ok = false;
            if (!L.up(m->rope_sin, sn.data(), sn.size() * 4)) L.ok = false;
        }
    }
    hipStreamSynchronize(L.s);
    if (L.stage) hipFree(L.stage);
    if (!stream) hipStreamDestroy(L.s);
    if (!L.ok) {
        model_free(m);
        return nullptr;
    }
    return m;
}

void model_free(Model* m) {
    if (!m) return;
    for (void* d : m->allocs) hipFree(d);
    delete m;
}

int kv_alloc(KVCache& kv, int n_layers, int n_slots, int n_kv, int n_ctx, hipStream_t s) {
    kv.n_layers = n_layers;
    kv.n_slots = n_slots;
    kv.n_kv = n_kv;
    kv.n_ctx = n_ctx;
    const size_t bytes = kv.layer_stride() * n_layers * sizeof(half_t);
    Q3_HIP(hipMalloc((void**)&kv.k, bytes), -1);
    Q3_HIP(hipMalloc((void**)&kv.v, bytes), -1);
    Q3_HIP(hipMemsetAsync(kv.k, 0, bytes, s), -1);
    Q3_HIP(hipMemsetAsync(kv.v, 0, bytes, s), -1);
    Q3_HIP(hipStreamSynchronize(s), -1);
    return 0;
}
void kv_free(KVCache& kv) {
    if (kv.k) hipFree(kv.k);
    if (kv.v) hipFree(kv.v);
    kv.k = kv.v = nullptr;
}

int kv_zero(hipStream_t s, KVCache& kv) {
    const size_t bytes = kv.layer_stride() * kv.n_layers * sizeof(half_t);
    Q3_HIP(hipMemsetAsync(kv.k, 0, bytes, s), -1);
    Q3_HIP(hipMemsetAsync(kv.v, 0, bytes, s), -1);
    return 0;
}

int work_zero(hipStream_t s, Work& w, const ModelCfg& c, int ffn, int max_vocab) {
    const size_t R = (size_t)w.max_rows;
    const int qkv_ld = (c.n_heads + 2 * c.n_kv) * c.head_dim;
    Q3_HIP(hipMemsetAsync(w.rows_in, 0, R * c.hidden * 4, s), -1);
    Q3_HIP(hipMemsetAsync(w.h, 0, R * c.hidden * 4, s), -1);
    Q3_HIP(hipMemsetAsync(w.ssq, 0, R * (c.hidden / 16) * 4, s), -1);
    Q3_HIP(hipMemsetAsync(w.xh, 0, R * c.hidden * 2, s), -1);
    Q3_HIP(hipMemsetAsync(w.qkv, 0, R * qkv_ld * 4, s), -1);
    Q3_HIP(hipMemsetAsync(w.attn, 0, R * c.n_heads * c.head_dim * 2, s), -1);
    Q3_HIP(hipMemsetAsync(w.act, 0, R * ffn * 2, s), -1);
    Q3_HIP(hipMemsetAsync(w.hidden_f32, 0, R * c.hidden * 4, s), -1);
    Q3_HIP(hipMemsetAsync(w.hidden_f16, 0, R * c.hidden * 2, s), -1);
    Q3_HIP(hipMemsetAsync(w.logits, 0, R * max_vocab * 4, s), -1);
    return 0;
}

int work_alloc(Work& w, const ModelCfg& c, int max_rows, int ffn, int max_vocab, hipStream_t s) {
    max_rows = (max_rows + 127) / 128 * 128;
    w.max_rows = max_rows;
    w.hidden = c.hidden;
    const size_t R = (size_t)max_rows;
    const int qkv_ld = (c.n_heads + 2 * c.n_kv) * c.head_dim;
    Q3_HIP(hipMalloc((void**)&w.rows_in, R * c.hidden * 4), -1);
    Q3_HIP(hipMalloc((void**)&w.h, R * c.hidden * 4), -1);
    Q3_HIP(hipMemsetAsync(w.h, 0, R * c.hidden * 4, s), -1);
    Q3_HIP(hipMalloc((void**)&w.ssq, R * (c.hidden / 16) * 4), -1);
    Q3_HIP(hipMalloc((void**)&w.xh, R * c.hidden * 2), -1);
    Q3_HIP(hipMemsetAsync(w.xh, 0, R * c.hidden * 2, s), -1);
    Q3_HIP(hipMalloc((void**)&w.qkv, R * qkv_ld * 4), -1);
    Q3_HIP(hipMalloc((void**)&w.attn, R * c.n_heads * c.head_dim * 2), -1);
    Q3_HIP(hipMemsetAsync(w.attn, 0, R * c.n_heads * c.head_dim * 2, s), -1);
    Q3_HIP(hipMalloc((void**)&w.act, R * ffn * 2), -1);
    Q3_HIP(hipMemsetAsync(w.act, 0, R * ffn * 2, s), -1);
    Q3_HIP(hipMalloc((void**)&w.hidden_f32, R * c.hidden * 4), -1);
    Q3_HIP(hipMalloc((void**)&w.hidden_f16, R * c.hidden * 2), -1);
    Q3_HIP(hipMemsetAsync(w.hidden_f16, 0, R * c.hidden * 2, s), -1);
    Q3_HIP(hipMalloc((void**)&w.logits, R * max_vocab * 4), -1);
    Q3_HIP(hipMalloc((void**)&w.map_slot, R * 4), -1);
    Q3_HIP(hipMalloc((void**)&w.map_pos, R * 4), -1);
    Q3_HIP(hipStreamSynchronize(s), -1);
    w.map_R16 = 0;
    return 0;
}
void work_free(Work& w) {
    void* ps[] = {w.rows_in, w.h, w.ssq, w.xh, w.qkv, w.attn, w.act, w.hidden_f32, w.hidden_f16, w.logits, w.map_slot, w.map_pos};
    for (void* p : ps)
        if (p) hipFree(p);
    w = Work();
}

int run_stack(hipStream_t s, const Model& m, const DevStack& st, Work& w, KVCache& kv, int R, const RowMap& rm,
              int attn_threads, int row0) {
    const ModelCfg& c = m.cfg;
    const int H = c.hidden, D = c.head_dim;
    const int qkv_ld = (c.n_heads + 2 * c.n_kv) * D;
    if (row0 % 16) {
        Q3_LOG("run_stack: row0=%d must be a multiple of 16 (fragment-ordered activations)", row0);
        return -1;
    }
    if (row0 + R > w.max_rows) {
        Q3_LOG("run_stack: %d rows > workspace %d", R, w.max_rows);
        return -1;
    }
    for (size_t li = 0; li < st.L.size(); li++) {
        const DevLayer& L = st.L[li];
        LinArgs a;
        a = LinArgs();
        a.wp = L.qkv.wp;
        a.N = L.qkv.N;
        a.K = H;
        a.M = row0 + R;
        a.m_begin = row0;
        a.nt = st.nt;
        a.x16 = w.xh;
        a.ssq = w.ssq;
        a.ssq_parts = H / 16;
        a.eps = c.eps;
        a.y = w.qkv;
        a.ldy = qkv_ld;
        if (!(li == 0 && rm.skip_qkv0) && launch_linear(s, a, PRO_NORM, EPI_STORE)) return -1;
        AttnArgs t;
        t.qkv = w.qkv;
        t.ld = qkv_ld;
        t.R = R;
        t.row0 = row0;
        t.q_norm = L.q_norm;
        t.k_norm = L.k_norm;
        t.eps = c.eps;
        t.rope_cos = m.rope_cos;
        t.rope_sin = m.rope_sin;
        t.slot = rm.slot;
        t.pos = rm.pos;
        t.slot_base = rm.slot_base;
        t.slot_stride = rm.slot_stride;
        t.pos_base = rm.pos_base;
        t.pos_stride = rm.pos_stride;
        t.kc = kv.k + li * kv.layer_stride();
        t.vc = kv.v + li * kv.layer_stride();
        t.n_ctx = kv.n_ctx;
        t.n_kv = c.n_kv;
        t.n_heads = c.n_heads;
        t.out = w.attn;
        t.scale = 1.0f / sqrtf((float)D);
        t.threads = attn_threads;
        if (rm.rows_total > R) {
            const int fit = 65536 / (rm.rows_total * c.n_kv);
            if (t.threads > fit) t.threads = fit / 64 * 64;
            if (t.threads < 256) t.threads = 256;
        }
        t.valid_mod = rm.valid_mod;
        t.valid_n = rm.valid_n;
        if (rm.same_slot_rows && R > 1) {
            if (launch_attn(s, t, ATTN_PREP)) return -1;
            if (rm.tiles && rm.n_tiles > 0) {
                t.tiles = rm.tiles;
                t.n_tiles = rm.n_tiles;
            } else if (!rm.slot && !rm.pos && rm.slot_stride == 0 && rm.pos_stride == 1 && rm.valid_mod == 0) {
                t.tiles = nullptr;
                t.n_tiles = (R + 15) / 16;
            }
            if (launch_attn(s, t, ATTN_ATTEND)) return -1;
        } else {
            if (launch_attn(s, t, ATTN_FUSED)) return -1;
        }
        a = LinArgs();
        a.wp = L.o.wp;
        a.N = H;
        a.K = L.o.K;
        a.M = row0 + R;
        a.m_begin = row0;
        a.nt = st.nt;
        a.x16 = w.attn;
        a.h_out = w.h;
        a.ssq_out = w.ssq;
        a.xh_out = w.xh;
        a.gamma = L.post_ln;
        if (launch_linear(s, a, PRO_F16, EPI_RESID)) return -1;
        a = LinArgs();
        a.wp = L.gu.wp;
        a.N = L.gu.N;
        a.K = H;
        a.M = row0 + R;
        a.m_begin = row0;
        a.nt = st.nt;
        a.x16 = w.xh;
        a.ssq = w.ssq;
        a.ssq_parts = H / 16;
        a.eps = c.eps;
        a.act = w.act;
        if (launch_linear(s, a, PRO_NORM, EPI_SWIGLU)) return -1;
        a = LinArgs();
        a.wp = L.down.wp;
        a.N = H;
        a.K = L.down.K;
        a.M = row0 + R;
        a.m_begin = row0;
        a.nt = st.nt;
        a.x16 = w.act;
        a.h_out = w.h;
        a.ssq_out = w.ssq;
        a.gamma = li + 1 < st.L.size() ? st.L[li + 1].in_ln : st.tail_gamma;
        a.xh_out = a.gamma ? w.xh : nullptr;
        if (launch_linear(s, a, PRO_F16, EPI_RESID)) return -1;
    }
    return 0;
}

void GraphExec::reset() {
    if (e) hipGraphExecDestroy(e);
    if (g) hipGraphDestroy(g);
    e = nullptr;
    g = nullptr;
}

}
```

qwen3_tts_axera_russian_amd/csrc/q3_test_api.hip:

```cpp
#include "q3_enc.h"
#include "q3_model.h"
#include "q3_voc_ops.h"
#include <chrono>
#include <cstring>
#include <vector>

using namespace q3;

namespace q3 {
int set_linear_tuning(int K, int mt16, int kbw);
int set_linear_split_rows(int on);
int set_linear_narrow8(int on);
int set_linear_wide_tiles(int on);
int set_attn_short(int on);
int set_gemm_min_rows(int n);
int set_gemm_glds(int on);
int reset_linear_knobs();
const char* last_linear_variant();
}

namespace {
struct DBuf {
    void* p = nullptr;
    ~DBuf() {
// ... 141 lines not shown
        Q3_HIP(hipMemcpy(pro_ssq, dssq.p, (size_t)M * (K / 16) * 4, hipMemcpyDeviceToHost), -1);
        for (int m = 0; m < M; m++)
            for (int k = 0; k < K; k++) {
                pro_h[(size_t)m * K + k] = hpz[frag_idx_host(m, k, K)];
                pro_xh[(size_t)m * K + k] = xp[frag_idx_host(m, k, K)];
            }
        a.x16 = (const half_t*)dx.p;
        a.ssq = (const float*)dssq.p;
        a.ssq_parts = K / 16;
        a.eps = eps;
    }
    std::vector<uint32_t> hy, hh, hs;
    std::vector<uint16_t> hx, ha;
    if (epi == EPI_STORE) {
        hy.assign((size_t)Mp * ldy, GUARD32);
        if (!dy.up(hy.data(), hy.size() * 4)) return -1;
        a.y = (float*)dy.p;
        a.ldy = ldy;
    } else if (epi == EPI_RESID) {
        hh.assign((size_t)Mp * N, GUARD32);
        hs.assign((size_t)Mp * (N / 16), GUARD32);
        for (int m = m_begin; m < M; m++)
            for (int n = 0; n < N; n++) memcpy(&hh[frag_idx_host(m, n, N)], &h_io[(size_t)m * N + n], 4);
        if (!dho.up(hh.data(), hh.size() * 4) || !dso.up(hs.data(), hs.size() * 4)) return -1;
        a.h_out = (float*)dho.p;
        a.ssq_out = (float*)dso.p;
        if (xh_out) {
            hx.assign((size_t)Mp * N, GUARD16);
            if (!dxo.up(hx.data(), hx.size() * 2) || !dgn.up(gamma_next, (size_t)N * 4)) return -1;
            a.xh_out = (half_t*)dxo.p;
            a.gamma = (const float*)dgn.p;
        }
    } else {
        ha.assign((size_t)Mp * NA, GUARD16);
        if (!dact.up(ha.data(), ha.size() * 2)) return -1;
        a.act = (half_t*)dact.p;
    }
    Q3_HIP(hipDeviceSynchronize(), -1);
    if (launch_linear(s, a, pro, epi)) {
        if (!last_linear_variant()[0] && hipGetLastError() == hipSuccess) return -2;
        return -1;
    }
    Q3_HIP(hipDeviceSynchronize(), -1);
    auto inside = [&](int m) { return m >= m_begin && m < M; };
    int outside = 0;
    if (epi == EPI_STORE) {
        Q3_HIP(hipMemcpy(hy.data(), dy.p, hy.size() * 4, hipMemcpyDeviceToHost), -1);
        for (int m = 0; m < Mp; m++)
            for (int n = 0; n < ldy; n++) {
                const uint32_t v = hy[(size_t)m * ldy + n];
                if (inside(m) && n < N) memcpy(&y[(size_t)m * ldy + n], &v, 4);
                else if (v != GUARD32) outside++;
            }
    } else if (epi == EPI_RESID) {
        Q3_HIP(hipMemcpy(hh.data(), dho.p, hh.size() * 4, hipMemcpyDeviceToHost), -1);
        Q3_HIP(hipMemcpy(hs.data(), dso.p, hs.size() * 4, hipMemcpyDeviceToHost), -1);
        if (xh_out) Q3_HIP(hipMemcpy(hx.data(), dxo.p, hx.size() * 2, hipMemcpyDeviceToHost), -1);
        for (int m = 0; m < Mp; m++) {
            for (int n = 0; n < N; n++) {
                const size_t fi = frag_idx_host(m, n, N);
                if (inside(m)) {
                    memcpy(&h_io[(size_t)m * N + n], &hh[fi], 4);
                    if (xh_out) xh_out[(size_t)m * N + n] = hx[fi];
                } else if (hh[fi] != GUARD32 || (xh_out && hx[fi] != GUARD16)) {
                    outside++;
                }
            }
            for (int p = 0; p < N / 16; p++) {
                const uint32_t v = hs[(size_t)m * (N / 16) + p];
                if (inside(m)) memcpy(&ssq_out[(size_t)m * (N / 16) + p], &v, 4);
                else if (v != GUARD32) outside++;
            }
        }
    } else {
        Q3_HIP(hipMemcpy(ha.data(), dact.p, ha.size() * 2, hipMemcpyDeviceToHost), -1);
        for (int m = 0; m < Mp; m++)
            for (int j = 0; j < NA; j++) {
                const uint16_t v = ha[frag_idx_host(m, j, NA)];
                if (inside(m)) act[(size_t)m * NA + j] = v;
                else if (v != GUARD16) outside++;
            }
    }
    return outside ? -3 : 0;
}

int q3t_attn(int mode, int R, int row0, const float* qkv, const float* q_norm, const float* k_norm, float eps,
             const float* rope_cos, const float* rope_sin, int max_pos, const int* slot, const int* pos, int slot_base,
             int slot_stride, int pos_base, int pos_stride, uint16_t* kc, uint16_t* vc, int n_slots, int n_ctx,
             const int* tiles, int n_tiles, int valid_mod, int valid_n, int threads, uint16_t* out) {
    constexpr int NH = 16, NKV = 8, D = 128, LD = (NH + 2 * NKV) * D, OW = NH * D;
    constexpr uint16_t GUARD = 0x7d5au;
    if (mode != 0 && mode != 1) return -2;
    if (R <= 0 || row0 < 0 || !qkv || !q_norm || !k_norm || !rope_cos || !rope_sin || !kc || !vc || !out) return -2;
    if (max_pos <= 0 || n_slots <= 0 || n_ctx <= 0 || threads < 64 || threads > 1024 || threads % 64) return -2;
    if (valid_mod < 0 || (valid_mod > 0 && (valid_n < 0 || valid_n > valid_mod))) return -2;
    const int rows = row0 + R;
    auto skipped = [&](int r) { return valid_mod > 0 && (r % valid_mod) >= valid_n; };
    auto row_slot = [&](int r) { return slot ? slot[r - row0] : slot_base + r * slot_stride; };
    auto row_pos = [&](int r) { return pos ? pos[r - row0] : pos_base + r * pos_stride; };
    for (int r = row0; r < rows; r++) {
        if (skipped(r)) continue;
        const int sl = row_slot(r), p = row_pos(r);
        if (sl < 0 || sl >= n_slots || p < 0 || p >= n_ctx || p >= max_pos) return -2;
    }
    if (mode == 0) {
        if (n_tiles != 0 || tiles) return -2;
        std::vector<char> seen((size_t)n_slots, 0);
        for (int r = row0; r < rows; r++) {
            if (skipped(r)) continue;
            if (seen[(size_t)row_slot(r)]++) return -2;
        }
    } else if (n_tiles > 0 && !tiles) {
        if (slot || pos || slot_stride != 0 || pos_stride != 1 || valid_mod != 0 || n_tiles != (R + 15) / 16) return -2;
    } else if (n_tiles > 0) {
        for (int i = 0; i < n_tiles; i++) {
            const int* t = tiles + 4 * i;
            if (t[0] < row0 || t[1] < 1 || t[1] > 16 || t[0] + t[1] > rows) return -2;
            if (t[2] < 0 || t[2] >= n_slots || t[3] < 0 || t[3] + t[1] > n_ctx) return -2;
        }
    } else if (n_tiles < 0 || tiles) {
        return -2;
    }
    hipStream_t s = nullptr;
    const int Rp = (rows + 15) / 16 * 16;
    const size_t cache = (size_t)n_slots * NKV * n_ctx * D;
    std::vector<float> hq((size_t)Rp * LD, 0.f);
    memcpy(hq.data() + (size_t)row0 * LD, qkv, (size_t)R * LD * 4);
    std::vector<uint16_t> ho((size_t)Rp * OW, GUARD);
    for (int r = row0; r < rows; r++)
        for (int k = 0; k < OW; k++) ho[frag_idx_host(r, k, OW)] = out[(size_t)(r - row0) * OW + k];
    std::vector<int> hs((size_t)Rp, 0), hp((size_t)Rp, 0);
    for (int r = row0; r < rows; r++) {
        if (slot) hs[r] = slot[r - row0];
        if (pos) hp[r] = pos[r - row0];
    }
    DBuf dq, dqn, dkn, dcs, dsn, dkc, dvc, dout, dslot, dpos, dtiles;
    if (!dq.up(hq.data(), hq.size() * 4) || !dqn.up(q_norm, D * 4) || !dkn.up(k_norm, D * 4) ||
        !dcs.up(rope_cos, (size_t)max_pos * 64 * 4) || !dsn.up(rope_sin, (size_t)max_pos * 64 * 4) ||
        !dkc.up(kc, cache * 2) || !dvc.up(vc, cache * 2) || !dout.up(ho.data(), ho.size() * 2) ||
        !dslot.up(hs.data(), hs.size() * 4) || !dpos.up(hp.data(), hp.size() * 4))
        return -1;
    if (tiles && !dtiles.up(tiles, (size_t)n_tiles * 16)) return -1;
    AttnArgs t;
    t.qkv = (float*)dq.p;
    t.ld = LD;
    t.R = R;
    t.row0 = row0;
    t.q_norm = (const float*)dqn.p;
    t.k_norm = (const float*)dkn.p;
    t.eps = eps;
    t.rope_cos = (const float*)dcs.p;
    t.rope_sin = (const float*)dsn.p;
    t.slot = slot ? (const int*)dslot.p : nullptr;
    t.pos = pos ? (const int*)dpos.p : nullptr;
    t.slot_base = slot_base;
    t.slot_stride = slot_stride;
    t.pos_base = pos_base;
    t.pos_stride = pos_stride;
    t.kc = (half_t*)dkc.p;
    t.vc = (half_t*)dvc.p;
    t.n_ctx = n_ctx;
    t.n_kv = NKV;
    t.n_heads = NH;
    t.out = (half_t*)dout.p;
    t.scale = 1.0f / sqrtf((float)D);
    t.threads = threads;
// ... 283 lines not shown
```

qwen3_tts_axera_russian_amd/engine.py:

```python
from __future__ import annotations

import math
from dataclasses import dataclass

import numpy as np

from . import hiplib


@dataclass(frozen=True)
class SlotParams:
    max_frames: int
    temperature: float = 0.0
    top_k: int = 50
    top_p: float = 1.0
    cp_temperature: float = 0.0
    cp_top_k: int = 50
    seed: int = 0
    utt: int = 0

    def check(self, max_frames):
        for name in ("temperature", "cp_temperature"):
            v = getattr(self, name)
            if not (isinstance(v, (int, float)) and math.isfinite(v) and v >= 0):
                raise ValueError(f"{name} must be finite and >= 0 (got {v!r})")
        if not (isinstance(self.top_p, (int, float)) and 0 < self.top_p <= 1):
            raise ValueError(f"top_p must be in (0, 1] (got {self.top_p!r})")
        for name in ("max_frames", "top_k", "cp_top_k", "seed", "utt"):
            if isinstance(getattr(self, name), bool) or not isinstance(getattr(self, name), (int, np.integer)):
                raise ValueError(f"{name} must be an integer (got {getattr(self, name)!r})")
        if not 1 <= self.max_frames <= max_frames:
            raise ValueError(f"max_frames must be in 1..{max_frames} (got {self.max_frames})")
        if not 0 <= self.seed < 1 << 64:
            raise ValueError(f"seed must fit in a u64 (got {self.seed})")
        if not 0 <= self.utt < 1 << 31:
            raise ValueError(f"utt must be in 0..2**31-1 (got {self.utt})")
        if not (-(1 << 31) <= self.top_k < 1 << 31 and -(1 << 31) <= self.cp_top_k < 1 << 31):
            raise ValueError("top_k / cp_top_k must fit in an i32")


class FrameEngine:
    def __init__(self, weights_path, max_batch=32, n_ctx=512, max_frames=256):
        self._lib = hiplib.load()
        self.h = self._lib.q3e_create(str(weights_path).encode(), max_batch, n_ctx, max_frames)
        if not self.h:
            raise RuntimeError(f"q3e_create failed: {weights_path}")
        self.max_batch, self.n_ctx, self.max_frames = max_batch, n_ctx, max_frames
        self.B = 0
        self.frame_steps = 0

    def set_sampling(self, talker_temperature=0.0, talker_top_k=50, talker_top_p=0.95, cp_temperature=0.0,
                     cp_top_k=50, seed=0):
        if self._lib.q3e_set_sampling(self.h, float(talker_temperature), int(talker_top_k), float(talker_top_p),
                                      float(cp_temperature), int(cp_top_k), int(seed)) != 0:
            raise RuntimeError("q3e_set_sampling failed")

    def set_chains(self, n):
        if self._lib.q3e_set_chains(self.h, int(n)) != 0:
            raise RuntimeError("q3e_set_chains failed")

    def set_pad_embed(self, pad):
        pad = np.ascontiguousarray(pad, dtype=np.float32).reshape(-1)
        if self._lib.q3e_set_pad_embed(self.h, hiplib.fptr(pad)) != 0:
            raise RuntimeError("q3e_set_pad_embed failed")

    def start(self, prefixes, n_text, ignore_eos=False, max_frames=0):
        n_rows = np.array([p.shape[0] for p in prefixes], np.int32)
        cat = np.ascontiguousarray(np.concatenate(prefixes, axis=0), dtype=np.float32)
        nt = np.ascontiguousarray(n_text, dtype=np.int32)
        self.B = len(prefixes)
        rc = self._lib.q3e_start(self.h, self.B, hiplib.fptr(cat), hiplib.iptr(n_rows), hiplib.iptr(nt),
                                 int(bool(ignore_eos)), int(max_frames))
        if rc != 0:
            raise RuntimeError(f"q3e_start failed: {rc}")

    def set_forced_codes(self, forced):
        if forced is None:
            rc = self._lib.q3e_set_forced_codes(self.h, None, 0)
        else:
            f = np.ascontiguousarray(forced, dtype=np.int32)
            assert f.ndim == 3 and f.shape[1] == self.B and f.shape[2] == 16
            rc = self._lib.q3e_set_forced_codes(self.h, hiplib.iptr(f), f.shape[0])
        if rc != 0:
            raise RuntimeError("q3e_set_forced_codes failed")

    def run(self, n_frames):
        rc = self._lib.q3e_run(self.h, int(n_frames))
        if rc < 0:
            raise RuntimeError(f"q3e_run failed: {rc}")
        self.frame_steps += rc
        return rc

    @property
    def last_run_ms(self):
        return float(self._lib.q3e_last_run_ms(self.h))

    @property
    def last_prefill_ms(self):
        return float(self._lib.q3e_last_prefill_ms(self.h))

    @property
    def step_weight_bytes(self):
        return float(self._lib.q3e_step_weight_bytes(self.h))

    def codes(self):
        out = np.full((self.max_frames, self.B, 16), -1, np.int32)
        per = np.zeros(self.B, np.int32)
        nf = self._lib.q3e_get_codes(self.h, hiplib.iptr(out), self.max_frames, hiplib.iptr(per))
        if nf < 0:
            raise RuntimeError("q3e_get_codes failed")
        return out[:nf], per

    def done(self):
        d = np.zeros(self.B, np.int32)
        per = np.zeros(self.B, np.int32)
        if self._lib.q3e_get_done(self.h, hiplib.iptr(d), hiplib.iptr(per)) != 0:
            raise RuntimeError("q3e_get_done failed")
        return d.astype(bool), per

    def refill(self, slots, prefixes, n_text):
        slots = np.ascontiguousarray(np.asarray(slots, np.int32))
        assert len(slots) == len(prefixes) == len(n_text) and len(slots) > 0
        cat = np.ascontiguousarray(np.concatenate([np.asarray(p, np.float32) for p in prefixes], axis=0))
        n_rows = np.array([p.shape[0] for p in prefixes], np.int32)
        nt = np.ascontiguousarray(np.asarray(n_text, np.int32))
        rc = self._lib.q3e_refill(self.h, len(slots), hiplib.iptr(slots), hiplib.fptr(cat), hiplib.iptr(n_rows), hiplib.iptr(nt))
        if rc != 0:
            raise RuntimeError(f"q3e_refill failed: {rc}")

    def generate_queue(self, prefixes, n_text, max_frames, ignore_eos=False, check_every=8, on_done=None, on_frames=None):
        n = len(prefixes)
        assert n == len(n_text) and n > 0
        B = min(self.max_batch, n)
        out = [None] * n
        owner = list(range(B))
        nxt = B
        self.start(prefixes[:B], n_text[:B], ignore_eos=ignore_eos, max_frames=max_frames)
        while any(o is not None for o in owner):
            ran = self.run(check_every)
            done, per = self.done()
            fin = [b for b in range(B) if owner[b] is not None and (done[b] or per[b] >= max_frames)]
            codes = None
            if on_frames is not None:
                codes, _ = self.codes()
                on_frames(codes, per, list(owner), fin)
            if not fin:
                if ran == 0:
                    raise RuntimeError("generate_queue: the engine ran no frame and no utterance finished")
                continue
            if codes is None:
                codes, _ = self.codes()
            for b in fin:
                res = np.ascontiguousarray(codes[:int(per[b]), b, :])
                out[owner[b]] = res
                if on_done is not None:
                    on_done(owner[b], res)
                owner[b] = None
            take = [b for b in fin if nxt + fin.index(b) < n]
            if take:
                idx = [nxt + i for i in range(len(take))]
                self.refill(take, [prefixes[i] for i in idx], [n_text[i] for i in idx])
                for b, i in zip(take, idx):
                    owner[b] = i
                nxt += len(take)
        return out

    def open(self, B=None, ignore_eos=False):
        B = self.max_batch if B is None else int(B)
        if self._lib.q3e_open(self.h, B, int(bool(ignore_eos))) != 0:
            raise RuntimeError("q3e_open failed")
        self.B = B

    def admit(self, slots, prefixes, n_text, params):
        slots = np.ascontiguousarray(np.asarray(slots, np.int32))
        assert len(slots) == len(prefixes) == len(n_text) == len(params) and len(slots) > 0
        for p in params:
            p.check(self.max_frames)
        cat = np.ascontiguousarray(np.concatenate([np.asarray(p, np.float32) for p in prefixes], axis=0))
# ... 26 lines not shown
```

qwen3_tts_axera_russian_amd/hiplib.py:

```python
from __future__ import annotations

import ctypes
import os

from . import LIB_PATH, TEST_LIB_PATH

_lib = None
_test_lib = None

c_void_p, c_int, c_float, c_char_p = ctypes.c_void_p, ctypes.c_int, ctypes.c_float, ctypes.c_char_p
f32p = ctypes.POINTER(ctypes.c_float)
i32p = ctypes.POINTER(ctypes.c_int32)
i64p = ctypes.POINTER(ctypes.c_int64)
u16p = ctypes.POINTER(ctypes.c_uint16)
i16p = ctypes.POINTER(ctypes.c_int16)


class SlotParamsC(ctypes.Structure):
    _fields_ = [("max_frames", ctypes.c_int32), ("temperature", ctypes.c_float), ("top_k", ctypes.c_int32),
                ("top_p", ctypes.c_float), ("cp_temperature", ctypes.c_float), ("cp_top_k", ctypes.c_int32),
                ("seed", ctypes.c_uint64), ("utt", ctypes.c_int32), ("reserved", ctypes.c_int32)]


def _sig(lib, name, restype, argtypes):
    fn = getattr(lib, name)
    fn.restype, fn.argtypes = restype, argtypes


def load(path: str | None = None):
    global _lib
    if _lib is not None and path is None:
        return _lib
    p = path or os.environ.get("QWEN3TTS_LIB", LIB_PATH)
    if not os.path.exists(p):
        raise RuntimeError(f"{p} not found: build it with `python -m qwen3_tts_axera_russian_amd.build` "
                           "(the HIP library is the only compute path)")
    if os.environ.get("Q3_KEEP_HW_QUEUES", "0") in ("", "0"):
        os.environ.setdefault("GPU_MAX_HW_QUEUES", "1")
    lib = ctypes.CDLL(p)
    _sig(lib, "wrapper_backend_init", None, [])
    _sig(lib, "wrapper_backend_free", None, [])
    _sig(lib, "wrapper_load_model", c_void_p, [c_char_p, c_int])
    _sig(lib, "wrapper_free_model", None, [c_void_p])
    _sig(lib, "wrapper_model_n_embd", c_int, [c_void_p])
    _sig(lib, "wrapper_create_context", c_void_p, [c_void_p, c_int, c_int, c_int, c_int])
    _sig(lib, "wrapper_create_context_slots", c_void_p, [c_void_p, c_int, c_int, c_int])
    _sig(lib, "wrapper_free_context", None, [c_void_p])
    _sig(lib, "wrapper_ctx_n_slots", c_int, [c_void_p])
    _sig(lib, "wrapper_kv_clear", None, [c_void_p])
    _sig(lib, "wrapper_decode_embd", c_int, [c_void_p, f32p, c_int, c_int, c_int, f32p])
    _sig(lib, "wrapper_decode_embd_slot", c_int, [c_void_p, c_int, f32p, c_int, c_int, c_int, f32p])
    _sig(lib, "wrapper_decode_embd_batch", c_int, [c_void_p, f32p, c_int, c_int, i32p, i32p, f32p])
    _sig(lib, "wrapper_codec_head", c_int, [c_void_p, f32p, c_int, f32p])
    _sig(lib, "wrapper_state_get_size", ctypes.c_size_t, [c_void_p])
    _sig(lib, "wrapper_state_save_file", c_int, [c_void_p, c_char_p])
    _sig(lib, "wrapper_state_load_file", c_int, [c_void_p, c_char_p])
    _sig(lib, "cp_load", c_void_p, [c_char_p, c_char_p, c_int])
    _sig(lib, "cp_free", None, [c_void_p])
    _sig(lib, "cp_hidden_size", c_int, [c_void_p])
    _sig(lib, "cp_predict", c_int, [c_void_p, f32p, ctypes.c_int32, c_float, c_int, ctypes.c_uint64, i32p])
    _sig(lib, "cp_predict_batch", c_int, [c_void_p, f32p, i32p, c_int, c_float, c_int, ctypes.c_uint64, i32p])
    _sig(lib, "cp_step", c_int, [c_void_p, f32p, c_int, f32p])
    _sig(lib, "cp_lm_head", c_int, [c_void_p, c_int, f32p, f32p])
    _sig(lib, "q3e_create", c_void_p, [c_char_p, c_int, c_int, c_int])
    _sig(lib, "q3e_free", None, [c_void_p])
    _sig(lib, "q3e_set_pad_embed", c_int, [c_void_p, f32p])
    _sig(lib, "q3e_set_chains", c_int, [c_void_p, c_int])
    _sig(lib, "q3e_set_sampling", c_int, [c_void_p, c_float, c_int, c_float, c_float, c_int, ctypes.c_uint64])
    _sig(lib, "q3e_set_forced_codes", c_int, [c_void_p, i32p, c_int])
    _sig(lib, "q3e_start", c_int, [c_void_p, c_int, f32p, i32p, i32p, c_int, c_int])
    _sig(lib, "q3e_run", c_int, [c_void_p, c_int])
    _sig(lib, "q3e_last_run_ms", c_float, [c_void_p])
    _sig(lib, "q3e_last_prefill_ms", c_float, [c_void_p])
    _sig(lib, "q3e_get_codes", c_int, [c_void_p, i32p, c_int, i32p])
    _sig(lib, "q3e_get_done", c_int, [c_void_p, i32p, i32p])
    _sig(lib, "q3e_refill", c_int, [c_void_p, c_int, i32p, f32p, i32p, i32p])
    _sig(lib, "q3e_open", c_int, [c_void_p, c_int, c_int])
    _sig(lib, "q3e_admit", c_int, [c_void_p, c_int, i32p, f32p, i32p, i32p, ctypes.POINTER(SlotParamsC)])
    _sig(lib, "q3e_release", c_int, [c_void_p, c_int, i32p])
    _sig(lib, "q3e_get_hidden", c_int, [c_void_p, f32p])
    _sig(lib, "q3e_step_weight_bytes", ctypes.c_double, [c_void_p])
    _sig(lib, "voc_load", c_void_p, [c_char_p, c_int, c_int])
    _sig(lib, "voc_free", None, [c_void_p])
    _sig(lib, "voc_chunk_tokens", c_int, [c_void_p])
    _sig(lib, "voc_samples_per_token", c_int, [c_void_p])
    _sig(lib, "voc_chunk_samples", c_int, [c_void_p])
    _sig(lib, "voc_decode", c_int, [c_void_p, i64p, c_int, f32p])
    _sig(lib, "voc_synthesize", c_int, [c_void_p, i64p, c_int, i16p, i32p])
    _sig(lib, "voc_synthesize_f32", c_int, [c_void_p, i64p, c_int, f32p, i32p])
    _sig(lib, "voc_synthesize_max_samples", c_int, [c_void_p, c_int])
    _sig(lib, "voc_set_max_workgroups", c_int, [c_int])
    _sig(lib, "voc_set_exact_fp32", c_int, [c_int])
    _sig(lib, "voc_set_fused_units", c_int, [c_int])
    _sig(lib, "voc_last_decode_ms", c_float, [c_void_p])
    _sig(lib, "voc_decode_flops", ctypes.c_double, [c_void_p, c_int])
    i64p_ = ctypes.POINTER(ctypes.c_int64)
    _sig(lib, "voc_synthesize_batch", c_int, [c_void_p, i64p, i32p, c_int, i16p, ctypes.c_int64, i64p_])
    _sig(lib, "voc_synthesize_batch_f32", c_int, [c_void_p, i64p, i32p, c_int, f32p, ctypes.c_int64, i64p_])
    _sig(lib, "voc_synthesize_batch_max_samples", ctypes.c_int64, [c_void_p, i32p, c_int])
    _sig(lib, "voc_last_batch_ms", c_float, [c_void_p])
    _sig(lib, "voc_last_batch_chunks", c_int, [c_void_p])
    _sig(lib, "voc_stream_create", c_void_p, [c_void_p, c_int])
    _sig(lib, "voc_stream_free", None, [c_void_p])
    _sig(lib, "voc_stream_reset", c_int, [c_void_p, c_int])
    _sig(lib, "voc_stream_push_max_samples", ctypes.c_int64, [c_void_p, c_int, i32p, i32p, i32p])
    _sig(lib, "voc_stream_push", c_int, [c_void_p, c_int, i32p, i64p, i32p, i32p, i16p, ctypes.c_int64, i64p_])
    _sig(lib, "voc_stream_push_f32", c_int, [c_void_p, c_int, i32p, i64p, i32p, i32p, f32p, ctypes.c_int64, i64p_])
    _sig(lib, "voc_stream_last_decodes", c_int, [c_void_p])
    _sig(lib, "voc_stream_last_chunks", c_int, [c_void_p])
    _sig(lib, "voc_stream_last_ms", c_float, [c_void_p])
    _sig(lib, "voc_incr_create", c_void_p, [c_void_p, c_int])
    _sig(lib, "voc_incr_free", None, [c_void_p])
    _sig(lib, "voc_incr_reset", c_int, [c_void_p, c_int])
    _sig(lib, "voc_incr_push_max_samples", ctypes.c_int64, [c_void_p, c_int, i32p, i32p, i32p])
    _sig(lib, "voc_incr_push", c_int, [c_void_p, c_int, i32p, i64p, i32p, i32p, i16p, ctypes.c_int64, i64p_])
    _sig(lib, "voc_incr_push_f32", c_int, [c_void_p, c_int, i32p, i64p, i32p, i32p, f32p, ctypes.c_int64, i64p_])
    _sig(lib, "voc_incr_last_ms", c_float, [c_void_p])
    _sig(lib, "voc_incr_last_launches", c_int, [c_void_p])
    _sig(lib, "voc_incr_samples", ctypes.c_int64, [c_void_p, ctypes.c_int64])
    _sig(lib, "voc_incr_state_bytes", ctypes.c_int64, [c_void_p])
    _sig(lib, "voc_incr_device_bytes", ctypes.c_int64, [c_void_p])
    _sig(lib, "voc_incr_set_arithmetic", c_int, [c_void_p, c_int])
    _sig(lib, "voc_incr_arithmetic", c_int, [c_void_p])
    _sig(lib, "voc_incr_last_split_launches", c_int, [c_void_p])
    _sig(lib, "voc_incr_last_redone", c_int, [c_void_p])
    _sig(lib, "enc_load", c_void_p, [c_char_p, c_int, c_int])
    _sig(lib, "enc_free", None, [c_void_p])
    _sig(lib, "enc_num_quantizers", c_int, [c_void_p])
    _sig(lib, "enc_sample_rate", c_int, [c_void_p])
    _sig(lib, "enc_samples_per_frame", c_int, [c_void_p])
    _sig(lib, "enc_frames", c_int, [c_void_p, c_int])
    _sig(lib, "enc_encode", c_int, [c_void_p, f32p, i32p, c_int, i64p_, c_int, i32p])
    _sig(lib, "enc_last_ms", c_float, [c_void_p])
    _sig(lib, "enc_debug_shape", c_int, [c_void_p, i32p, c_int, c_int, i32p, i32p])
    _sig(lib, "enc_debug_run", c_int, [c_void_p, f32p, i32p, c_int, c_int, f32p, i32p, i32p])
    _sig(lib, "enc_stream_create", c_void_p, [c_void_p, c_int, c_int])
    _sig(lib, "enc_stream_free", None, [c_void_p])
    _sig(lib, "enc_stream_reset", c_int, [c_void_p, c_int])
    _sig(lib, "enc_stream_push_max_frames", c_int, [c_void_p, c_int, i32p, i32p, i32p])
    _sig(lib, "enc_stream_push", c_int, [c_void_p, c_int, i32p, f32p, i32p, i32p, i64p_, ctypes.c_int64, i64p_])
    _sig(lib, "enc_stream_last_ms", c_float, [c_void_p])
    _sig(lib, "enc_stream_last_launches", c_int, [c_void_p])
    _sig(lib, "enc_stream_state_bytes", ctypes.c_int64, [c_void_p])
    _sig(lib, "enc_stream_device_bytes", ctypes.c_int64, [c_void_p])
    _sig(lib, "tfe_load", c_void_p, [c_char_p, c_char_p, c_int])
    _sig(lib, "tfe_free", None, [c_void_p])
    _sig(lib, "tfe_hidden_size", c_int, [c_void_p])
    _sig(lib, "tfe_text_vocab", c_int, [c_void_p])
    _sig(lib, "tfe_embed_text", c_int, [c_void_p, i32p, c_int, f32p])
    _sig(lib, "tfe_build_prefix", c_int, [c_void_p, i32p, c_int, i32p, f32p])
    _sig(lib, "tfe_tts_pad_embed", c_int, [c_void_p, f32p])
    _sig(lib, "q3_device_count", c_int, [])
    _sig(lib, "q3_device_compute_units", c_int, [])
    _sig(lib, "q3_set_device", c_int, [c_int])
    if path is None:
        _lib = lib
    return lib


def load_test():
    global _test_lib
    if _test_lib is not None:
        return _test_lib
    load()
    if not os.path.exists(TEST_LIB_PATH):
        raise RuntimeError(f"{TEST_LIB_PATH} not found: build it with `python -m qwen3_tts_axera_russian_amd.build`")
    lib = ctypes.CDLL(TEST_LIB_PATH)
    _sig(lib, "q3t_set_linear_tuning", c_int, [c_int, c_int, c_int])
    _sig(lib, "q3t_linear", c_int, [c_int, c_int, c_int, u16p, c_int, c_int, c_int, u16p, f32p, f32p, c_float,
                                    f32p, f32p, u16p, c_int])
    _sig(lib, "q3t_linear_case", c_int, [c_int, c_int, c_int, c_int, u16p, c_int, c_int, c_int, c_int, c_float, c_int,
                                         u16p, f32p, f32p, f32p, f32p, f32p, u16p, f32p, f32p, f32p, u16p, u16p])
    _sig(lib, "q3t_reset_linear_knobs", c_int, [])
    _sig(lib, "q3t_last_linear_variant", c_char_p, [])
    _sig(lib, "q3t_talker_sample", c_int, [f32p, c_int, i32p, c_int, c_int, c_int])
    _sig(lib, "q3t_attn", c_int, [c_int, c_int, c_int, f32p, f32p, f32p, c_float, f32p, f32p, c_int, i32p, i32p, c_int,
                                  c_int, c_int, c_int, u16p, u16p, c_int, c_int, i32p, c_int, c_int, c_int, c_int, u16p])
    _sig(lib, "q3t_voc_attn", c_int, [c_int, f32p, f32p, c_int, c_int, c_int, c_int, c_int, c_float])
    _sig(lib, "q3t_set_linear_split_rows", c_int, [c_int])
    _sig(lib, "q3t_set_linear_narrow8", c_int, [c_int])
    _sig(lib, "q3t_set_linear_wide_tiles", c_int, [c_int])
    _sig(lib, "q3t_set_attn_short", c_int, [c_int])
    _sig(lib, "q3t_set_gemm_min_rows", c_int, [c_int])
    _sig(lib, "q3t_set_gemm_glds", c_int, [c_int])
    _sig(lib, "q3t_inspect_weights", c_int, [ctypes.c_char_p, ctypes.c_char_p, ctypes.c_char_p, c_int])
    _sig(lib, "q3t_bench_linear", c_float, [c_int, c_int, c_int, c_int, c_int, c_int, c_int, c_int])
    _sig(lib, "q3t_bench_chain", c_float, [c_int, c_int, c_int, c_int, c_int, c_int])
    _sig(lib, "q3t_cp_model_load", c_void_p, [c_char_p])
    _sig(lib, "q3t_cp_model_free", None, [c_void_p])
    _sig(lib, "q3t_cp_qkv_ld", c_int, [c_void_p])
    _sig(lib, "q3t_cp_qkv_serves", c_int, [c_void_p, c_int])
    _sig(lib, "q3t_cp_qkv_tab", c_int, [c_void_p, c_int, i32p, c_int, f32p])
    _sig(lib, "q3t_cp_qkv_live", c_int, [c_void_p, c_int, i32p, c_int, c_int, f32p])
    _sig(lib, "q3t_enc_stream_embeddings", c_int, [c_void_p, c_int, i32p, f32p, i32p, i32p, i64p, ctypes.c_int64, i64p, f32p, i32p])
    i64s = ctypes.POINTER(ctypes.c_longlong)
    _sig(lib, "q3t_enc_stream_plan", c_int, [i32p, i32p, c_int, ctypes.c_longlong, ctypes.c_longlong, c_int, i64s, i64s, i64s])
    _test_lib = lib
    return lib


def fptr(a):
    return a.ctypes.data_as(f32p)


def iptr(a):
    return a.ctypes.data_as(i32p)
```

Baseline: 10170 codec_frames/s.

## Fuse code-predictor argmax into LM-head epilogue and next attention prologue

```diff
diff --git a/include/qwen3tts_engine.h b/include/qwen3tts_engine.h
--- a/include/qwen3tts_engine.h
+++ b/include/qwen3tts_engine.h
@@ -31,6 +31,8 @@
 float q3e_last_run_ms(void* e);
 float q3e_last_prefill_ms(void* e);
 
+int q3e_graph_nodes(void* e);
+
 int q3e_get_codes(void* e, int32_t* out, int max_out_frames, int32_t* n_frames_per_utt);
 
 int q3e_get_done(void* e, int32_t* done , int32_t* frames );
diff --git a/qwen3_tts_axera_russian_amd/build.py b/qwen3_tts_axera_russian_amd/build.py
--- a/qwen3_tts_axera_russian_amd/build.py
+++ b/qwen3_tts_axera_russian_amd/build.py
@@ -24,7 +24,7 @@
 
 
 NO_SPILL = ("resunit_kernel", "linear_kernelILi1ELi1E", "linear_kernelILi1ELi2E", "linear_kernelILi2ELi1E",
-            "linear_kernelILi2ELi2E", "attn_kernel", "attn_short_kernel", "cp_argmax_kernel", "talker_sample_kernel",
+            "linear_kernelILi2ELi2E", "attn_kernel", "attn_short_kernel", "attn_short_cpf_kernel", "cp_argmax_kernel", "talker_sample_kernel",
             "voc_attn_incr_kernel", "voc_incr_prepend_kernel", "voc_incr_emit_kernel", "voc_incr_prepend_split_kernel",
             "enc_stream_conv_in_kernel", "enc_stream_unfold_kernel", "enc_stream_emit_kernel")
 
diff --git a/qwen3_tts_axera_russian_amd/csrc/q3_cp.h b/qwen3_tts_axera_russian_amd/csrc/q3_cp.h
--- a/qwen3_tts_axera_russian_amd/csrc/q3_cp.h
+++ b/qwen3_tts_axera_russian_amd/csrc/q3_cp.h
@@ -18,7 +18,9 @@
     const unsigned long long* seed_ptr = nullptr;
     const int* forced = nullptr;
     const SlotParams* slots = nullptr;
+    bool fuse_argmax = false;
 };
+bool cp_fused_argmax_enabled();
 
 int cp_seed_row0(const Work& w, int R, int row0 = 0, int R_total = 0);
 int cp_frame(hipStream_t s, const Model& m, Work& w, KVCache& kv, int R, const CpFrameIO& io, int row0 = 0,
diff --git a/qwen3_tts_axera_russian_amd/csrc/q3_cp_api.hip b/qwen3_tts_axera_russian_amd/csrc/q3_cp_api.hip
--- a/qwen3_tts_axera_russian_amd/csrc/q3_cp_api.hip
+++ b/qwen3_tts_axera_russian_amd/csrc/q3_cp_api.hip
@@ -5,6 +5,11 @@
 
 static bool two_row_enabled() {
     static const bool on = !(getenv("Q3_CP_TWO_ROW") && atoi(getenv("Q3_CP_TWO_ROW")) == 0);
+    return on;
+}
+
+bool cp_fused_argmax_enabled() {
+    static const bool on = !(getenv("Q3_CP_FUSED_ARGMAX") && atoi(getenv("Q3_CP_FUSED_ARGMAX")) == 0);
     return on;
 }
 
@@ -74,12 +79,19 @@
         if (run_stack(s, m, m.cp, w, kv, R, rm, 256, row0)) return -1;
     }
     const bool qkv_tab = m.cp_qkv_serves(R);
+    const int parts = linear_pmax_parts(H, c.cp_vocab, R);
+    const bool fuse = io.fuse_argmax && qkv_tab && !io.slots && !(io.temperature > 1e-6f) && H == 1024 && parts > 0 && parts <= 128 &&
+                      c.cp_vocab % 16 == 0;
+    CpFuseArgs cf;
+    bool fused_prev = false;
     for (int g = 0; g < G; g++) {
         if (g > 0) {
             rm.pos_base = g + 1;
             rm.skip_qkv0 = qkv_tab;
+            rm.cp_fuse0 = fused_prev ? &cf : nullptr;
             if (run_stack(s, m, m.cp, w, kv, R, rm, 256, row0)) return -1;
         }
+        const bool fuse_this = fuse && g + 1 < G && attn_short_takes(g + 2, kv.n_ctx);
         LinArgs a;
         a.wp = m.cp_head[g].wp;
         a.N = c.cp_vocab;
@@ -93,7 +105,29 @@
         a.eps = c.eps;
         a.y = w.logits;
         a.ldy = c.cp_vocab;
-        if (launch_linear(s, a, PRO_NORM, EPI_STORE)) return -1;
+        a.pmax = fuse_this ? w.pmax : nullptr;
+        if (launch_linear(s, a, PRO_NORM, fuse_this ? EPI_STORE_PMAX : EPI_STORE)) return -1;
+        fused_prev = fuse_this;
+        if (fuse_this) {
+            cf = CpFuseArgs();
+            cf.pmax = w.pmax;
+            cf.parts = parts;
+            cf.V = c.cp_vocab;
+            cf.H = H;
+            cf.group = g;
+            cf.R_total = R_total;
+            cf.frame_cap = io.frame_cap;
+            cf.codes = io.codes;
+            cf.n_frames = io.n_frames;
+            cf.forced = io.forced;
+            cf.table = m.cp_emb[g];
+            cf.qkv_tab = m.cp_qkv_rows(g);
+            cf.h_out = w.h;
+            cf.ssq_out = w.ssq;
+            cf.xh_out = w.xh;
+            cf.gamma_next = m.cp.L[0].in_ln;
+            continue;
+        }
         CpArgmaxArgs x;
         x.logits = w.logits;
         x.V = c.cp_vocab;
diff --git a/qwen3_tts_axera_russian_amd/csrc/q3_engine.hip b/qwen3_tts_axera_russian_amd/csrc/q3_engine.hip
--- a/qwen3_tts_axera_russian_amd/csrc/q3_engine.hip
+++ b/qwen3_tts_axera_russian_amd/csrc/q3_engine.hip
@@ -134,6 +134,7 @@
     io.seed_ptr = e->d_seed;
     io.forced = e->forced_on ? e->d_forced : nullptr;
     io.slots = e->slot_mode ? e->d_slots : nullptr;
+    io.fuse_argmax = cp_fused_argmax_enabled();
     if (cp_frame(st, m, e->wc, e->kv_c, R, io, row0, e->B)) return -1;
     RowMap rm;
     rm.slot_base = 0;
@@ -587,6 +588,25 @@
     return done_frames;
 }
 
+int q3e_graph_nodes(void* ee) {
+    Engine* e = (Engine*)ee;
+    if (!e) return -1;
+    size_t total = 0;
+    for (int c = 0; c < 8; c++) {
+        size_t n = 0;
+        if (!e->graph[c].g) continue;
+        if (hipGraphGetNodes(e->graph[c].g, nullptr, &n) != hipSuccess) return -1;
+        std::vector<hipGraphNode_t> nodes(n);
+        if (n && hipGraphGetNodes(e->graph[c].g, nodes.data(), &n) != hipSuccess) return -1;
+        for (size_t i = 0; i < n; i++) {
+            hipGraphNodeType ty;
+            if (hipGraphNodeGetType(nodes[i], &ty) != hipSuccess) return -1;
+            if (ty == hipGraphNodeTypeKernel) total++;
+        }
+    }
+    return (int)total;
+}
+
 float q3e_last_run_ms(void* ee) { return ee ? ((Engine*)ee)->last_run_ms : -1.f; }
 float q3e_last_host_launch_ms(void* ee) { return ee ? ((Engine*)ee)->last_host_launch_ms : -1.f; }
 float q3e_last_prefill_ms(void* ee) { return ee ? ((Engine*)ee)->last_prefill_ms : -1.f; }
diff --git a/qwen3_tts_axera_russian_amd/csrc/q3_kernels.h b/qwen3_tts_axera_russian_amd/csrc/q3_kernels.h
--- a/qwen3_tts_axera_russian_amd/csrc/q3_kernels.h
+++ b/qwen3_tts_axera_russian_amd/csrc/q3_kernels.h
@@ -4,7 +4,7 @@
 namespace q3 {
 
 enum { PRO_F16 = 0, PRO_NORM = 1 };
-enum { EPI_STORE = 0, EPI_RESID = 1, EPI_SWIGLU = 2 };
+enum { EPI_STORE = 0, EPI_RESID = 1, EPI_SWIGLU = 2, EPI_STORE_PMAX = 3 };
 
 struct LinArgs {
     int tl_node = -1;
@@ -24,8 +24,10 @@
     half_t* xh_out = nullptr;
     const float* gamma = nullptr;
     half_t* act = nullptr;
+    int2* pmax = nullptr;
 };
 int launch_linear(hipStream_t s, const LinArgs& a, int pro, int epi);
+int linear_pmax_parts(int K, int N, int rows);
 int linear_decode_kbw(int K, int N, int rows);
 
 int launch_pack_linear(hipStream_t s, const half_t* src, int N, int K, half_t* dst, int tile_off,
@@ -53,7 +55,23 @@
     int valid_mod = 0, valid_n = 0;
     const int* tiles = nullptr;
     int n_tiles = 0;
+    const struct CpFuseArgs* cp_fuse = nullptr;
 };
+struct CpFuseArgs {
+    const int2* pmax = nullptr;
+    int parts = 0;
+    int V = 0, H = 0, group = 0, R_total = 0, frame_cap = 0;
+    int* codes = nullptr;
+    const int* n_frames = nullptr;
+    const int* forced = nullptr;
+    const float* table = nullptr;
+    const float* qkv_tab = nullptr;
+    float* h_out = nullptr;
+    float* ssq_out = nullptr;
+    half_t* xh_out = nullptr;
+    const float* gamma_next = nullptr;
+};
+int attn_short_takes(int pos_base, int n_ctx);
 int launch_attn(hipStream_t s, const AttnArgs& a, int mode);
 
 int launch_ssq_rows(hipStream_t s, const float* rows, float* h, float* ssq, int R, int H, half_t* xh = nullptr,
diff --git a/qwen3_tts_axera_russian_amd/csrc/q3_kernels.hip b/qwen3_tts_axera_russian_amd/csrc/q3_kernels.hip
--- a/qwen3_tts_axera_russian_amd/csrc/q3_kernels.hip
+++ b/qwen3_tts_axera_russian_amd/csrc/q3_kernels.hip
@@ -5,6 +5,14 @@
 typedef _Float16 h8 __attribute__((ext_vector_type(8)));
 typedef float f4 __attribute__((ext_vector_type(4)));
 
+#ifndef Q3_WAVE_PRIO
+#define Q3_WAVE_PRIO 3
+#endif
+#if Q3_WAVE_PRIO > 0
+#define Q3_SETPRIO() __builtin_amdgcn_s_setprio(Q3_WAVE_PRIO)
+#else
+#define Q3_SETPRIO()
+#endif
 #ifdef Q3_TIMELINE
 __device__ unsigned long long* g_tl = nullptr;
 __device__ unsigned int g_tl_idx = 0;
@@ -43,6 +51,7 @@
     }
 };
 #define Q3_TL(id)      \
+    Q3_SETPRIO();       \
     if (g_skip) return; \
     TlScope2 tl_scope2_(a.tl_node, id); \
     TlScope tl_scope_(id)
@@ -51,14 +60,7 @@
         if (tl_scope_.slot < g_tl_cap && g_ph) g_ph[(size_t)tl_scope_.slot * 8 + (n)] = wall_clock64(); \
     } while (0)
 #else
-#ifndef Q3_WAVE_PRIO
-#define Q3_WAVE_PRIO 3
-#endif
-#if Q3_WAVE_PRIO > 0
-#define Q3_TL(id) __builtin_amdgcn_s_setprio(Q3_WAVE_PRIO)
-#else
-#define Q3_TL(id)
-#endif
+#define Q3_TL(id) Q3_SETPRIO()
 #define Q3_PH(n)
 #endif
 
@@ -78,6 +80,7 @@
     for (int o = 32; o > 0; o >>= 1) v = fmaxf(v, __shfl_xor(v, o, 64));
     return v;
 }
+__device__ __forceinline__ float nan_as_inf(float l);
 __device__ __forceinline__ half_t sat_half(float x) {
     return (half_t)fminf(fmaxf(x, -65504.f), 65504.f);
 }
@@ -126,7 +129,9 @@
 static const char* g_last_variant = "";
 const char* last_linear_variant() { return g_last_variant; }
 static const char* pro_name(int pro) { return pro == PRO_NORM ? "NORM" : "F16"; }
-static const char* epi_name(int epi) { return epi == EPI_STORE ? "STORE" : epi == EPI_RESID ? "RESID" : "SWIGLU"; }
+static const char* epi_name(int epi) {
+    return epi == EPI_STORE ? "STORE" : epi == EPI_RESID ? "RESID" : epi == EPI_SWIGLU ? "SWIGLU" : "STORE_PMAX";
+}
 static int env_int(const char* name, int dflt) { return getenv(name) ? atoi(getenv(name)) : dflt; }
 
 template <int NB16, int MT16, int KBW, int NW, int PRO, int EPI, bool NT>
@@ -151,6 +156,7 @@
     constexpr int NOUT = (EPI == EPI_SWIGLU) ? MR * NB / 2 : MR * NB;
     constexpr int OPT = (NOUT + NTH - 1) / NTH;
     constexpr int SQI = (MR * 16 + NTH - 1) / NTH;
+    constexpr bool STORE = EPI == EPI_STORE || EPI == EPI_STORE_PMAX;
     Q3_TL(10 + PRO * 4 + EPI);
     const int tid = threadIdx.x, lane = tid & 63, w = tid >> 6;
     const int q = lane >> 4, c = lane & 15;
@@ -200,6 +206,7 @@
     __builtin_amdgcn_sched_barrier(0);
     if (EPI == EPI_RESID) Q3_FETCH_ARGS("s"(a.ssq_out), "s"(a.xh_out));
     if (EPI == EPI_STORE) Q3_FETCH_ARGS("s"(a.ldy));
+    if (EPI == EPI_STORE_PMAX) Q3_FETCH_ARGS("s"(a.ldy), "s"(a.pmax));
     if (PRO == PRO_NORM) Q3_FETCH_ARGS("s"(a.eps));
     Q3_PH(0);
 
@@ -242,7 +249,7 @@
     __syncthreads();
     Q3_PH(3);
 
-    if (EPI == EPI_STORE || EPI == EPI_RESID) {
+    if (STORE || EPI == EPI_RESID) {
 #pragma unroll
         for (int i = 0; i < OPT; i++) {
             const int o = tid + i * NTH;
@@ -255,8 +262,22 @@
                 const int ng = tile0 * 16 + n;
                 const bool ok = m < a.M;
                 if (PRO == PRO_NORM) v *= inv_s[mr];
-                if (EPI == EPI_STORE) {
+                if (STORE) {
                     if (ok) Q3_OUT_STORE(v, &a.y[(size_t)m * a.ldy + ng]);
+                    if (EPI == EPI_STORE_PMAX) {
+                        float bv = nan_as_inf(v);
+                        int bi = ng;
+#pragma unroll
+                        for (int off = NB / 2; off > 0; off >>= 1) {
+                            const float ov = __shfl_xor(bv, off, NB);
+                            const int oi = __shfl_xor(bi, off, NB);
+                            if (ov > bv || (ov == bv && oi < bi)) {
+                                bv = ov;
+                                bi = oi;
+                            }
+                        }
+                        if (ok && n == 0) a.pmax[(size_t)m * (a.N / NB) + tile0 / NB16] = make_int2(__float_as_int(bv), bi);
+                    }
                 } else {
                     const float hn = ok ? hold[i] + v : 0.f;
                     if (ok) Q3_OUT_STORE(hn, &a.h_out[frag_idx(m, ng, a.N)]);
@@ -320,7 +341,7 @@
     b.swap_grid = nr_ > 2 ? 1 : 0;
     dim3 grid(b.swap_grid ? nr_ : nt_, b.swap_grid ? nt_ : nr_);
     const void* asrc = (const void*)b.x16;
-    void* outp = EPI == EPI_STORE ? (void*)b.y : EPI == EPI_RESID ? (void*)b.h_out : (void*)b.act;
+    void* outp = (EPI == EPI_STORE || EPI == EPI_STORE_PMAX) ? (void*)b.y : EPI == EPI_RESID ? (void*)b.h_out : (void*)b.act;
     hipLaunchKernelGGL((linear_kernel<NB16, MT16, KBW, NW, PRO, EPI, NT>), grid, dim3(NW * 64), lds, s, b.wp, asrc, b.ssq,
                        b.gamma, outp, b.M, b.N, b.m_begin, b.swap_grid, b.eps, b);
     Q3_HIP(hipGetLastError(), -1);
@@ -789,10 +810,33 @@
     return g_tune_kbw[ki][mt16 == 1 ? 0 : mt16 == 2 ? 1 : 2];
 }
 
+int linear_pmax_parts(int K, int N, int rows) {
+    if (!linear_decode_kbw(K, N, rows)) return 0;
+    return N / ((g_wide_tiles && rows > 16 && K == 1024) ? 32 : 16);
+}
+
+static int launch_linear_pmax(hipStream_t s, const LinArgs& a, int pro) {
+    const int rows = a.M - a.m_begin, K = a.K, epi = EPI_STORE_PMAX;
+    if (rows >= g_gemm_min_rows || pro != PRO_NORM || !a.pmax || K != 1024 || a.N % 32) {
+        Q3_LOG("launch_linear: the partial arg-max epilogue is built for the normed K = 1024 weight-streaming kernel only (%d rows)", rows);
+        return -1;
+    }
+    const int mt16 = decode_mt16(rows, a.N);
+    const int kbw = g_tune_kbw[0][mt16 == 1 ? 0 : mt16 == 2 ? 1 : 2];
+    const int nw = K / 32 / kbw;
+    const int nb16 = (g_wide_tiles && rows > 16) ? 2 : 1;
+    Q3_LIN_MT(1, 8, 4, PRO_NORM, EPI_STORE_PMAX)
+    Q3_LIN_MT(1, 4, 8, PRO_NORM, EPI_STORE_PMAX)
+    Q3_LIN_MT(2, 4, 8, PRO_NORM, EPI_STORE_PMAX)
+    Q3_LOG("launch_linear: no partial arg-max instantiation for kbw=%d nw=%d mt16=%d nb16=%d", kbw, nw, mt16, nb16);
+    return -1;
+}
+
 int launch_linear(hipStream_t s, const LinArgs& a, int pro, int epi) {
     g_last_variant = "";
     const int rows = a.M - a.m_begin;
     if (rows <= 0) return 0;
+    if (epi == EPI_STORE_PMAX) return launch_linear_pmax(s, a, pro);
     if (rows >= g_gemm_min_rows) return launch_gemm(s, a, pro, epi);
     const int K = a.K;
     int ki = K == 1024 ? 0 : K == 2048 ? 1 : K == 3072 ? 2 : -1;
@@ -826,6 +870,20 @@
     return -1;
 }
 
+__device__ __forceinline__ void store_row_ssq_g(float* h, float* ssq, int r, int H, int k4, float4 v, half_t* xh, float4 g) {
+    *(float4*)(h + frag_idx(r, k4 * 4, H)) = v;
+    if (xh) {
+        half_t* p = xh + frag_idx(r, k4 * 4, H);
+        p[0] = pre_scaled(v.x, g.x);
+        p[1] = pre_scaled(v.y, g.y);
+        p[2] = pre_scaled(v.z, g.z);
+        p[3] = pre_scaled(v.w, g.w);
+    }
+    float s = v.x * v.x + v.y * v.y + v.z * v.z + v.w * v.w;
+    s += __shfl_xor(s, 1, 4);
+    s += __shfl_xor(s, 2, 4);
+    if ((k4 & 3) == 0) ssq[(size_t)r * (H / 16) + (k4 >> 2)] = s;
+}
 __device__ __forceinline__ void store_row_ssq(float* h, float* ssq, int r, int H, int k4, float4 v,
                                               half_t* xh = nullptr, const float* gamma = nullptr) {
     *(float4*)(h + frag_idx(r, k4 * 4, H)) = v;
@@ -1144,25 +1202,17 @@
 constexpr int ATTN_SHORT_MAX_T = 15;
 static int g_attn_short = 1;
 int set_attn_short(int on) { g_attn_short = on; return 0; }
-__global__ void __launch_bounds__(256)
-    attn_short_kernel(float* __restrict__ p_qkv, int p_ld, int p_row0, int p_n_heads, int p_n_kv,
-                      const float* __restrict__ p_q_norm, const float* __restrict__ p_k_norm,
-                      const float* __restrict__ p_rope_cos, const float* __restrict__ p_rope_sin, int p_pos_base,
-                      int p_slot_base, AttnArgs a) {
+int attn_short_takes(int pos_base, int n_ctx) {
+    return g_attn_short && pos_base >= 0 && pos_base <= ATTN_SHORT_MAX_T && pos_base < n_ctx;
+}
+template <bool CPF>
+__device__ __forceinline__ void attn_short_body(AttnArgs& a, const CpFuseArgs& f) {
     constexpr int D = 128, NE = ATTN_SHORT_MAX_T + 1;
-    a.qkv = p_qkv;
-    a.ld = p_ld;
-    a.row0 = p_row0;
-    a.n_heads = p_n_heads;
-    a.n_kv = p_n_kv;
-    a.q_norm = p_q_norm;
-    a.k_norm = p_k_norm;
-    a.rope_cos = p_rope_cos;
-    a.rope_sin = p_rope_sin;
-    a.pos_base = p_pos_base;
-    a.slot_base = p_slot_base;
     Q3_FETCH_ARGS("s"(a.eps), "s"(a.slot), "s"(a.slot_stride), "s"(a.kc), "s"(a.vc), "s"(a.n_ctx), "s"(a.out), "s"(a.scale));
-    Q3_TL(33);
+    if constexpr (CPF)
+        Q3_FETCH_ARGS("s"(a.ld), "s"(f.V), "s"(f.H), "s"(f.group), "s"(f.R_total), "s"(f.frame_cap), "s"(f.codes), "s"(f.n_frames),
+                      "s"(f.forced), "s"(f.table), "s"(f.qkv_tab), "s"(f.h_out), "s"(f.ssq_out), "s"(f.xh_out), "s"(f.gamma_next));
+    Q3_TL(CPF ? 34 : 33);
     const int r = a.row0 + blockIdx.x, g = blockIdx.y;
     const int tid = threadIdx.x, lane = tid & 63, w = tid >> 6;
     const int slot = a.slot ? uniform_load(a.slot + r) : a.slot_base + r * a.slot_stride;
@@ -1176,12 +1226,23 @@
     const int l16 = tid & 15, grp = tid >> 4;
     const int hh = tid >> 7, d = tid & 127;
     float x0 = 0.f, x1 = 0.f, gm0 = 1.f, gm1 = 1.f, cs = 1.f, sn = 0.f;
+    int2 pm0 = make_int2(0, 0), pm1 = pm0;
+    int nf_r = 0;
+    float4 gnx = make_float4(0.f, 0.f, 0.f, 0.f);
+    if constexpr (CPF) {
+        const int2* pp = f.pmax + (size_t)r * f.parts;
+        pm0 = pp[lane < f.parts ? lane : 0];
+        pm1 = pp[lane + 64 < f.parts ? lane + 64 : 0];
+        nf_r = uniform_load(f.n_frames + r);
+        if (g == 0 && f.xh_out) gnx = *(const float4*)(f.gamma_next + tid * 4);
+    }
+    const size_t col = w < 2 ? (size_t)(2 * g + w) * D : w == 2 ? (size_t)(a.n_heads + g) * D : (size_t)(a.n_heads + a.n_kv + g) * D;
     {
-        const float* src = w < 2 ? row + (size_t)(2 * g + w) * D
-                         : w == 2 ? row + (size_t)(a.n_heads + g) * D
-                                  : row + (size_t)(a.n_heads + a.n_kv + g) * D;
-        x0 = src[lane];
-        x1 = src[lane + 64];
+        const float* src = row + col;
+        if constexpr (!CPF) {
+            x0 = src[lane];
+            x1 = src[lane + 64];
+        }
         if (w < 3) {
             const float* gam = w < 2 ? a.q_norm : a.k_norm;
             gm0 = gam[lane];
@@ -1194,6 +1255,54 @@
     if (grp < T) {
         kpre = *(const h8*)(a.kc + cbase + (size_t)grp * D + l16 * 8);
         vpre = *(const h8*)(a.vc + cbase + (size_t)grp * D + l16 * 8);
+    }
+    if constexpr (CPF) {
+        const int RT = f.R_total;
+        int f_idx = nf_r - 1, fzv = -1;
+        if (f_idx < 0) f_idx = 0;
+        const bool keep = f_idx < f.frame_cap;
+        if (!keep) f_idx = f.frame_cap - 1;
+        const size_t fo = ((size_t)f_idx * RT + r) * 16 + 1 + f.group;
+        if (f.forced && keep) fzv = uniform_load(f.forced + fo);
+        __builtin_amdgcn_sched_barrier(0);
+        float best = -INFINITY;
+        int bidx = 0x7fffffff;
+        if (lane < f.parts) {
+            best = __int_as_float(pm0.x);
+            bidx = pm0.y;
+        }
+        if (lane + 64 < f.parts) {
+            const float ov = __int_as_float(pm1.x);
+            if (ov > best || (ov == best && pm1.y < bidx)) {
+                best = ov;
+                bidx = pm1.y;
+            }
+        }
+#pragma unroll
+        for (int o = 32; o > 0; o >>= 1) {
+            const float ov = __shfl_xor(best, o, 64);
+            const int oi = __shfl_xor(bidx, o, 64);
+            if (ov > best || (ov == best && oi < bidx)) {
+                best = ov;
+                bidx = oi;
+            }
+        }
+        bidx = __builtin_amdgcn_readfirstlane(bidx);
+        if (bidx < 0 || bidx >= f.V) bidx = 0;
+        if (g == 0 && tid == 0 && keep) f.codes[fo] = bidx;
+        if (fzv >= 0) bidx = fzv;
+        const bool ok = bidx < f.V;
+        const int t = ok ? bidx : 0;
+        const float* src = f.qkv_tab + (size_t)t * a.ld + col;
+        x0 = src[lane];
+        x1 = src[lane + 64];
+        float4 ev = make_float4(0.f, 0.f, 0.f, 0.f);
+        if (g == 0) ev = *(const float4*)(f.table + (size_t)t * f.H + tid * 4);
+        if (!ok) {
+            x0 = x1 = 0.f;
+            ev = make_float4(0.f, 0.f, 0.f, 0.f);
+        }
+        if (g == 0) store_row_ssq_g(f.h_out, f.ssq_out, r, f.H, tid, ev, f.xh_out, gnx);
     }
     __builtin_amdgcn_sched_barrier(0);
     Q3_PH(0);
@@ -1268,6 +1377,42 @@
     }
     Q3_PH(3);
     a.out[frag_idx(r, (2 * g + hh) * D + d, a.n_heads * D)] = sat_half(o / L);
+}
+__global__ void __launch_bounds__(256)
+    attn_short_kernel(float* __restrict__ p_qkv, int p_ld, int p_row0, int p_n_heads, int p_n_kv,
+                      const float* __restrict__ p_q_norm, const float* __restrict__ p_k_norm,
+                      const float* __restrict__ p_rope_cos, const float* __restrict__ p_rope_sin, int p_pos_base,
+                      int p_slot_base, AttnArgs a) {
+    a.qkv = p_qkv;
+    a.ld = p_ld;
+    a.row0 = p_row0;
+    a.n_heads = p_n_heads;
+    a.n_kv = p_n_kv;
+    a.q_norm = p_q_norm;
+    a.k_norm = p_k_norm;
+    a.rope_cos = p_rope_cos;
+    a.rope_sin = p_rope_sin;
+    a.pos_base = p_pos_base;
+    a.slot_base = p_slot_base;
+    attn_short_body<false>(a, CpFuseArgs());
+}
+__global__ void __launch_bounds__(256)
+    attn_short_cpf_kernel(const int2* __restrict__ p_pmax, int p_parts, int p_row0, int p_n_heads, int p_n_kv,
+                          const float* __restrict__ p_q_norm, const float* __restrict__ p_k_norm,
+                          const float* __restrict__ p_rope_cos, const float* __restrict__ p_rope_sin, int p_pos_base,
+                          int p_slot_base, AttnArgs a, CpFuseArgs f) {
+    f.pmax = p_pmax;
+    f.parts = p_parts;
+    a.row0 = p_row0;
+    a.n_heads = p_n_heads;
+    a.n_kv = p_n_kv;
+    a.q_norm = p_q_norm;
+    a.k_norm = p_k_norm;
+    a.rope_cos = p_rope_cos;
+    a.rope_sin = p_rope_sin;
+    a.pos_base = p_pos_base;
+    a.slot_base = p_slot_base;
+    attn_short_body<true>(a, f);
 }
 
 __global__ void __launch_bounds__(256) attn_tile_mfma_kernel(AttnArgs a) {
@@ -1465,8 +1610,23 @@
         Q3_LOG("attn: only GQA group 2 (16q/8kv) is built, got %d/%d", a.n_heads, a.n_kv);
         return -1;
     }
-    if (g_attn_short && mode == ATTN_FUSED && !a.pos && a.pos_stride == 0 && a.pos_base >= 0 &&
-        a.pos_base <= ATTN_SHORT_MAX_T && a.pos_base < a.n_ctx) {
+    const bool take_short = mode == ATTN_FUSED && !a.pos && a.pos_stride == 0 && attn_short_takes(a.pos_base, a.n_ctx);
+    if (a.cp_fuse) {
+        const CpFuseArgs& f = *a.cp_fuse;
+        if (!take_short || f.H != 1024 || f.parts <= 0 || f.parts > 128 || !f.pmax || !f.qkv_tab || !f.table || !f.h_out ||
+            !f.ssq_out || !f.codes || !f.n_frames || f.R_total <= 0 || (f.xh_out && !f.gamma_next)) {
+            Q3_LOG("attn: the fused arg-max prologue needs the short-cache kernel, hidden 1024 and <= 128 pairs per row");
+            return -1;
+        }
+        AttnArgs a4 = a;
+        a4.tl_node = tl_next_node();
+        a4.cp_fuse = nullptr;
+        hipLaunchKernelGGL(attn_short_cpf_kernel, dim3(a.R, a.n_kv), dim3(256), 0, s, f.pmax, f.parts, a4.row0, a4.n_heads, a4.n_kv,
+                           a4.q_norm, a4.k_norm, a4.rope_cos, a4.rope_sin, a4.pos_base, a4.slot_base, a4, f);
+        Q3_HIP(hipGetLastError(), -1);
+        return 0;
+    }
+    if (take_short) {
         AttnArgs a3 = a;
         a3.tl_node = tl_next_node();
         hipLaunchKernelGGL(attn_short_kernel, dim3(a.R, a.n_kv), dim3(256), 0, s, a3.qkv, a3.ld, a3.row0, a3.n_heads, a3.n_kv,
diff --git a/qwen3_tts_axera_russian_amd/csrc/q3_model.h b/qwen3_tts_axera_russian_amd/csrc/q3_model.h
--- a/qwen3_tts_axera_russian_amd/csrc/q3_model.h
+++ b/qwen3_tts_axera_russian_amd/csrc/q3_model.h
@@ -72,6 +72,7 @@
     float* hidden_f32 = nullptr;
     half_t* hidden_f16 = nullptr;
     float* logits = nullptr;
+    int2* pmax = nullptr;
     int *map_slot = nullptr, *map_pos = nullptr;
     int map_R16 = 0;
 };
@@ -88,6 +89,7 @@
     const int* tiles = nullptr;
     int n_tiles = 0;
     bool skip_qkv0 = false;
+    const CpFuseArgs* cp_fuse0 = nullptr;
     int rows_total = 0;
 };
 
diff --git a/qwen3_tts_axera_russian_amd/csrc/q3_model.hip b/qwen3_tts_axera_russian_amd/csrc/q3_model.hip
--- a/qwen3_tts_axera_russian_amd/csrc/q3_model.hip
+++ b/qwen3_tts_axera_russian_amd/csrc/q3_model.hip
@@ -355,6 +355,8 @@
     Q3_HIP(hipMalloc((void**)&w.hidden_f16, R * c.hidden * 2), -1);
     Q3_HIP(hipMemsetAsync(w.hidden_f16, 0, R * c.hidden * 2, s), -1);
     Q3_HIP(hipMalloc((void**)&w.logits, R * max_vocab * 4), -1);
+    Q3_HIP(hipMalloc((void**)&w.pmax, R * (max_vocab / 16) * sizeof(int2)), -1);
+    Q3_HIP(hipMemsetAsync(w.pmax, 0, R * (max_vocab / 16) * sizeof(int2), s), -1);
     Q3_HIP(hipMalloc((void**)&w.map_slot, R * 4), -1);
     Q3_HIP(hipMalloc((void**)&w.map_pos, R * 4), -1);
     Q3_HIP(hipStreamSynchronize(s), -1);
@@ -362,7 +364,7 @@
     return 0;
 }
 void work_free(Work& w) {
-    void* ps[] = {w.rows_in, w.h, w.ssq, w.xh, w.qkv, w.attn, w.act, w.hidden_f32, w.hidden_f16, w.logits, w.map_slot, w.map_pos};
+    void* ps[] = {w.rows_in, w.h, w.ssq, w.xh, w.qkv, w.attn, w.act, w.hidden_f32, w.hidden_f16, w.logits, w.pmax, w.map_slot, w.map_pos};
     for (void* p : ps)
         if (p) hipFree(p);
     w = Work();
@@ -429,6 +431,13 @@
         }
         t.valid_mod = rm.valid_mod;
         t.valid_n = rm.valid_n;
+        if (li == 0 && rm.cp_fuse0) {
+            if (!rm.skip_qkv0 || (rm.same_slot_rows && R > 1)) {
+                Q3_LOG("run_stack: the fused arg-max needs a table-fed layer 0 with one position per row");
+                return -1;
+            }
+            t.cp_fuse = rm.cp_fuse0;
+        }
         if (rm.same_slot_rows && R > 1) {
             if (launch_attn(s, t, ATTN_PREP)) return -1;
             if (rm.tiles && rm.n_tiles > 0) {
diff --git a/qwen3_tts_axera_russian_amd/csrc/q3_test_api.hip b/qwen3_tts_axera_russian_amd/csrc/q3_test_api.hip
--- a/qwen3_tts_axera_russian_amd/csrc/q3_test_api.hip
+++ b/qwen3_tts_axera_russian_amd/csrc/q3_test_api.hip
@@ -247,6 +247,50 @@
             }
     }
     return outside ? -3 : 0;
+}
+
+int q3t_cp_head_partials(int M, int N, const uint16_t* W, const float* h, const float* gamma, float eps, float* y, float* pv,
+                         int* pi, int max_parts) {
+    constexpr int K = 1024;
+    if (M <= 0 || N <= 0 || N % 32 || !W || !h || !gamma || !y || !pv || !pi) return -2;
+    const int parts = linear_pmax_parts(K, N, M);
+    if (parts <= 0 || parts > max_parts) return -2;
+    hipStream_t s = nullptr;
+    const int Mp = (M + 127) / 128 * 128;
+    DBuf dW, dWp, dhrows, dh, dssq, dg, dxh, dy, dp;
+    if (!dW.up(W, (size_t)N * K * 2) || !dWp.alloc((size_t)N * K * 2)) return -1;
+    if (launch_pack_linear(s, (const half_t*)dW.p, N, K, (half_t*)dWp.p, 0, 1)) return -1;
+    if (!dhrows.up(h, (size_t)M * K * 4) || !dh.alloc((size_t)Mp * K * 4) || !dssq.alloc((size_t)Mp * (K / 16) * 4) ||
+        !dg.up(gamma, (size_t)K * 4) || !dxh.alloc((size_t)Mp * K * 2) || !dy.alloc((size_t)M * N * 4) ||
+        !dp.alloc((size_t)Mp * parts * sizeof(int2)))
+        return -1;
+    Q3_HIP(hipMemset(dh.p, 0, (size_t)Mp * K * 4), -1);
+    Q3_HIP(hipMemset(dssq.p, 0, (size_t)Mp * (K / 16) * 4), -1);
+    Q3_HIP(hipMemset(dxh.p, 0, (size_t)Mp * K * 2), -1);
+    Q3_HIP(hipMemset(dp.p, 0xff, (size_t)Mp * parts * sizeof(int2)), -1);
+    if (launch_ssq_rows(s, (const float*)dhrows.p, (float*)dh.p, (float*)dssq.p, M, K, (half_t*)dxh.p, (const float*)dg.p)) return -1;
+    LinArgs a;
+    a.wp = (const half_t*)dWp.p;
+    a.N = N;
+    a.K = K;
+    a.M = M;
+    a.x16 = (const half_t*)dxh.p;
+    a.ssq = (const float*)dssq.p;
+    a.ssq_parts = K / 16;
+    a.eps = eps;
+    a.y = (float*)dy.p;
+    a.ldy = N;
+    a.pmax = (int2*)dp.p;
+    if (launch_linear(s, a, PRO_NORM, EPI_STORE_PMAX)) return -1;
+    Q3_HIP(hipDeviceSynchronize(), -1);
+    Q3_HIP(hipMemcpy(y, dy.p, (size_t)M * N * 4, hipMemcpyDeviceToHost), -1);
+    std::vector<int2> hp((size_t)M * parts);
+    Q3_HIP(hipMemcpy(hp.data(), dp.p, hp.size() * sizeof(int2), hipMemcpyDeviceToHost), -1);
+    for (size_t i = 0; i < hp.size(); i++) {
+        memcpy(&pv[i], &hp[i].x, 4);
+        pi[i] = hp[i].y;
+    }
+    return parts;
 }
 
 int q3t_attn(int mode, int R, int row0, const float* qkv, const float* q_norm, const float* k_norm, float eps,
diff --git a/qwen3_tts_axera_russian_amd/engine.py b/qwen3_tts_axera_russian_amd/engine.py
--- a/qwen3_tts_axera_russian_amd/engine.py
+++ b/qwen3_tts_axera_russian_amd/engine.py
@@ -94,6 +94,10 @@
     @property
     def last_run_ms(self):
         return float(self._lib.q3e_last_run_ms(self.h))
+
+    @property
+    def graph_nodes(self):
+        return int(self._lib.q3e_graph_nodes(self.h))
 
     @property
     def last_prefill_ms(self):
diff --git a/qwen3_tts_axera_russian_amd/hiplib.py b/qwen3_tts_axera_russian_amd/hiplib.py
--- a/qwen3_tts_axera_russian_amd/hiplib.py
+++ b/qwen3_tts_axera_russian_amd/hiplib.py
@@ -71,6 +71,7 @@
     _sig(lib, "q3e_start", c_int, [c_void_p, c_int, f32p, i32p, i32p, c_int, c_int])
     _sig(lib, "q3e_run", c_int, [c_void_p, c_int])
     _sig(lib, "q3e_last_run_ms", c_float, [c_void_p])
+    _sig(lib, "q3e_graph_nodes", c_int, [c_void_p])
     _sig(lib, "q3e_last_prefill_ms", c_float, [c_void_p])
     _sig(lib, "q3e_get_codes", c_int, [c_void_p, i32p, c_int, i32p])
     _sig(lib, "q3e_get_done", c_int, [c_void_p, i32p, i32p])
@@ -192,6 +193,7 @@
     _sig(lib, "q3t_cp_qkv_serves", c_int, [c_void_p, c_int])
     _sig(lib, "q3t_cp_qkv_tab", c_int, [c_void_p, c_int, i32p, c_int, f32p])
     _sig(lib, "q3t_cp_qkv_live", c_int, [c_void_p, c_int, i32p, c_int, c_int, f32p])
+    _sig(lib, "q3t_cp_head_partials", c_int, [c_int, c_int, u16p, f32p, f32p, c_float, f32p, f32p, i32p, c_int])
     _sig(lib, "q3t_enc_stream_embeddings", c_int, [c_void_p, c_int, i32p, f32p, i32p, i32p, i64p, ctypes.c_int64, i64p, f32p, i32p])
     i64s = ctypes.POINTER(ctypes.c_longlong)
     _sig(lib, "q3t_enc_stream_plan", c_int, [i32p, i32p, c_int, ctypes.c_longlong, ctypes.c_longlong, c_int, i64s, i64s, i64s])
```

After: 10260 codec_frames/s, median of 6. Within noise of the previous version (+0.9%).
